# Chen-Suyi/PointRegGPT

Measured on AMD Instinct MI355X. Metric: generated point-cloud pairs/sec (node), 128x128 depth, 1000-step DDNM, higher is better.
Workload: dtype bf16; 1 GPU; configs[2]: full pipeline (SE(3) z-buffer reproject + MaskUnet + DDNM sampler + MaskUnet + f64 unproject); batch_per_gpu=64, image_size=128, transitions=1000, sampler=ancestral-ddnm, unet_dim=64, streams=2, parallelism=scene-sharded x1, no collectives, hipgraph=one captured transition (U-Net + update), replayed per step

## Files before the change

### include/prg.h

```cpp
#ifndef PRG_H
#define PRG_H

#include <stddef.h>
#include <stdint.h>

#ifdef __cplusplus
extern "C" {
#endif

#define PRG_ABI_VERSION 1

enum {
  PRG_OK = 0,
  PRG_E_INVALID = -1,
  PRG_E_HIP = -2,
  PRG_E_NOMEM = -3,
  PRG_E_STATE = -4
};

enum { PRG_F32 = 0, PRG_BF16 = 1, PRG_MXFP8 = 2, PRG_F16X3 = 3 };

int prg_abi_version(void);
const char* prg_last_error(void);
int prg_device_info(char* name, size_t name_len, int* compute_units);


int prg_depth2pc(const float* depth, const float* K, float* pc, uint8_t* valid, int B, int H, int W,
                 float clip_lo, float clip_hi, float invalid_value, void* stream);

int prg_pc2depth(const float* pc, const uint8_t* valid, const float* K, float* depth, uint8_t* mask,
                 int B, int N, int H, int W, void* stream);

int prg_project_points_zbuffer(const float* points, const int64_t* offsets, const float* pose, const float* K,
                               float* depth, uint8_t* mask, int B, int H, int W, float depth_scale,
                               void* stream);

int prg_reproject_zbuffer(const float* depth, const float* K, const float* pose, float* depth_out,
                          uint8_t* mask_out, int B, int H, int W, float depth_unit, float clip_lo,
                          float clip_hi, float out_scale, void* stream);

int prg_unproject_f64(const float* depth, const float* K, const float* pose, double* xyz, uint8_t* valid,
                      int B, int H, int W, float depth_unit, float clip_lo, float clip_hi, void* stream);

int prg_depth_augment(const float* depth, float* out, int B, int H, int W, void* stream);

int prg_apply_mask(const float* prob, const float* depth, const uint8_t* hit, float thr, float* depth_out,
                   uint8_t* hit_out, float* img_cond, int B, int H, int W, void* stream);

int prg_occlusion_filter(const float* depth, const uint8_t* mask, float* out, int B, int H, int W, float threshold,
                         void* stream);

int prg_overlap_counts(const double* pts, const int64_t* offsets, int n_pairs, int64_t max_cloud, double radius,
                       int32_t* counts, void* stream);

size_t prg_voxel_grid_workspace_bytes(int64_t total, int B);

int prg_voxel_grid_ragged(const double* pts, const uint8_t* valid, const int64_t* offsets, int B, int64_t total,
                          double voxel, double* out, int64_t* out_offsets, int32_t* status, void* workspace,
                          size_t workspace_bytes, void* stream);

int prg_merge_memory_f64(const float* memory, const int64_t* memory_offsets, int64_t memory_rows, const double* xyz,
                         const uint8_t* valid, int B, int HW, double* merged, uint8_t* merged_valid,
                         int64_t* merged_offsets, void* stream);


typedef struct prg_unet prg_unet;

typedef struct prg_unet_config {
  int32_t dim;
  int32_t n_levels;
  int32_t dim_mults[8];
  int32_t in_channels;
  int32_t conditional;
  int32_t param_cond_dim;
  int32_t groups;
  int32_t sigmoid_out;
} prg_unet_config;

int64_t prg_unet_param_count(const prg_unet_config* cfg);

int prg_unet_create(const prg_unet_config* cfg, const float* weights, int64_t n_floats, int dtype,
                    prg_unet** out);
int prg_unet_destroy(prg_unet* h);
int prg_unet_set_time_freqs(prg_unet* h, const float* freqs, int n);
int prg_unet_reserve(prg_unet* h, int B, int S);

int prg_unet_forward(prg_unet* h, const float* x, const int64_t* time, const float* param_cond, float* out,
                     int B, int S, void* stream);
int prg_maskunet_forward(prg_unet* h, const float* depth, float* prob, int B, int S, void* stream);

int prg_unet_set_taps(prg_unet* h, int enable);
int prg_unet_get_tap(prg_unet* h, const char* name, float* out, int64_t out_capacity_floats, int* C, int* H,
                     int* W, void* stream);

int prg_debug_conv3x3(const float* x, const float* w, const float* bias, float* out, int B, int Cin, int Cout, int H, int W,
                      int dtype, void* stream);
int prg_debug_block_pair(const float* x, const float* w1, const float* b1, const float* gamma, const float* beta, const float* w2,
                         const float* b2, float* out, int B, int Cin, int C, int H, int W, int groups, int h16, void* stream);
int prg_debug_upsample_conv3x3(const float* x, const float* w, const float* bias, float* out, int B, int Cin, int Cout, int H,
                               int W, void* stream);
int prg_debug_conv4x4s2(const float* x, const float* w, const float* bias, float* out, int B, int Cin, int Cout, int H, int W,
                        void* stream);
int prg_debug_conv(const float* x, const float* w, const float* bias, float* out, int B, int Cin, int Cout, int H, int W,
                   int dtype, int K, int stride, void* stream);
int prg_debug_upsample_conv(const float* x, const float* w, const float* bias, float* out, int B, int Cin, int Cout, int H, int W,
                            int dtype, void* stream);


typedef struct prg_sampler prg_sampler;

typedef struct prg_step {
  int32_t t;
  int32_t clip_pred;
  float c_x0, c_x, c_eps, sigma;
  float sqrt_recip, sqrt_recipm1;
} prg_step;

int prg_sampler_create(prg_unet* unet, const prg_step* steps, int n_steps, int B, int S, prg_sampler** out);
int prg_sampler_destroy(prg_sampler* h);
int prg_sampler_set_graph(prg_sampler* h, int enable);

int prg_sampler_run(prg_sampler* h, const float* param_cond, const float* img_cond, const float* noise,
                    int64_t noise_slabs, const uint64_t* seeds, float* out, void* stream);

int prg_debug_sampler_step(float* x, const float* u, const float* img_cond, const uint64_t* seeds, const prg_step* step, int B,
                           int HW, int reps, float* avg_us, void* stream);

int prg_sampler_set_profile(prg_sampler* h, int enable);
int prg_sampler_get_profile(prg_sampler* h, double* conv_ms, int64_t* conv_launches, double* conv_flops,
                            double* total_ms);
int prg_sampler_get_profile_bytes(prg_sampler* h, double* conv_bytes);
int prg_sampler_get_profile_executed(prg_sampler* h, double* conv_flops_executed);
typedef struct prg_profile_shape {
  int32_t cin, cout, k, stride, ups, hout, wout;
  int32_t two_source, prologue;
  int32_t mx;
  int64_t launches;
  double ms, flops, flops_executed;
} prg_profile_shape;
int prg_sampler_get_profile_shapes(prg_sampler* h, prg_profile_shape* rows, int32_t max_rows, int32_t* n_rows);
int prg_sampler_get_profile_step(prg_sampler* h, double* step_ms, int64_t* step_launches);


int prg_host_crop_aabb(const double* pts, int64_t n, const double* lo, const double* hi, double* out, int64_t* n_out);
int prg_host_voxel_down_sample(const double* pts, int64_t n, double voxel, double* out, int64_t* n_out);
int prg_host_write_ply(const char* path, const double* pts, int64_t n);

typedef struct prg_pool prg_pool;
int prg_pool_create(int n_threads, prg_pool** out);
int prg_pool_destroy(prg_pool* p);
int prg_pool_wait(prg_pool* p, int64_t* jobs_done);
int prg_pool_submit_cloud(prg_pool* p, const char* path, const double* xyz, int64_t n, const uint8_t* valid,
                          const double* T_pre, int crop, const double* lo, const double* hi, double voxel,
                          const double* T_post);
int prg_pool_submit_image(prg_pool* p, const char* path, const float* img, int H, int W, int kind);
int prg_pool_submit_text(prg_pool* p, const char* path, const double* values, int rows, int cols);

#ifdef __cplusplus
}
#endif
#endif
```

### pointreggpt_amd/_lib.py

```python
from __future__ import annotations

import ctypes as C
import os
from pathlib import Path

_HERE = Path(__file__).resolve().parent
LIB_PATH = Path(os.environ.get("PRG_HIP_LIB", _HERE / "libprg_hip.so"))

PRG_F32, PRG_BF16, PRG_MXFP8, PRG_F16X3 = 0, 1, 2, 3


class PrgError(RuntimeError):
    pass


class UnetConfigC(C.Structure):
    _fields_ = [("dim", C.c_int32), ("n_levels", C.c_int32), ("dim_mults", C.c_int32 * 8),
                ("in_channels", C.c_int32), ("conditional", C.c_int32), ("param_cond_dim", C.c_int32),
                ("groups", C.c_int32), ("sigmoid_out", C.c_int32)]


class StepC(C.Structure):
    _fields_ = [("t", C.c_int32), ("clip_pred", C.c_int32), ("c_x0", C.c_float), ("c_x", C.c_float),
                ("c_eps", C.c_float), ("sigma", C.c_float), ("sqrt_recip", C.c_float),
                ("sqrt_recipm1", C.c_float)]


_P, _I, _F, _L = C.c_void_p, C.c_int, C.c_float, C.c_int64

PROTOTYPES = {
    "prg_abi_version": (C.c_int, []),
    "prg_last_error": (C.c_char_p, []),
    "prg_device_info": (C.c_int, [C.c_char_p, C.c_size_t, C.POINTER(C.c_int)]),
    "prg_depth2pc": (C.c_int, [_P, _P, _P, _P, _I, _I, _I, _F, _F, _F, _P]),
    "prg_pc2depth": (C.c_int, [_P, _P, _P, _P, _P, _I, _I, _I, _I, _P]),
    "prg_project_points_zbuffer": (C.c_int, [_P, _P, _P, _P, _P, _P, _I, _I, _I, _F, _P]),
    "prg_reproject_zbuffer": (C.c_int, [_P, _P, _P, _P, _P, _I, _I, _I, _F, _F, _F, _F, _P]),
    "prg_unproject_f64": (C.c_int, [_P, _P, _P, _P, _P, _I, _I, _I, _F, _F, _F, _P]),
    "prg_depth_augment": (C.c_int, [_P, _P, _I, _I, _I, _P]),
    "prg_apply_mask": (C.c_int, [_P, _P, _P, _F, _P, _P, _P, _I, _I, _I, _P]),
    "prg_occlusion_filter": (C.c_int, [_P, _P, _P, _I, _I, _I, _F, _P]),
    "prg_overlap_counts": (C.c_int, [_P, _P, _I, _L, C.c_double, _P, _P]),
    "prg_voxel_grid_workspace_bytes": (C.c_size_t, [_L, _I]),
    "prg_voxel_grid_ragged": (C.c_int, [_P, _P, _P, _I, _L, C.c_double, _P, _P, _P, _P, C.c_size_t, _P]),
    "prg_merge_memory_f64": (C.c_int, [_P, _P, _L, _P, _P, _I, _I, _P, _P, _P, _P]),
    "prg_unet_param_count": (_L, [C.POINTER(UnetConfigC)]),
    "prg_unet_create": (C.c_int, [C.POINTER(UnetConfigC), _P, _L, _I, C.POINTER(_P)]),
    "prg_unet_destroy": (C.c_int, [_P]),
    "prg_unet_reserve": (C.c_int, [_P, _I, _I]),
    "prg_unet_set_time_freqs": (C.c_int, [_P, _P, _I]),
    "prg_unet_forward": (C.c_int, [_P, _P, _P, _P, _P, _I, _I, _P]),
    "prg_maskunet_forward": (C.c_int, [_P, _P, _P, _I, _I, _P]),
    "prg_debug_conv3x3": (C.c_int, [_P, _P, _P, _P, _I, _I, _I, _I, _I, _I, _P]),
    "prg_debug_block_pair": (C.c_int, [_P, _P, _P, _P, _P, _P, _P, _P, _I, _I, _I, _I, _I, _I, _I, _P]),
    "prg_debug_upsample_conv3x3": (C.c_int, [_P, _P, _P, _P, _I, _I, _I, _I, _I, _P]),
    "prg_debug_conv4x4s2": (C.c_int, [_P, _P, _P, _P, _I, _I, _I, _I, _I, _P]),
    "prg_debug_conv": (C.c_int, [_P, _P, _P, _P, _I, _I, _I, _I, _I, _I, _I, _I, _P]),
    "prg_debug_upsample_conv": (C.c_int, [_P, _P, _P, _P, _I, _I, _I, _I, _I, _I, _P]),
    "prg_unet_set_taps": (C.c_int, [_P, _I]),
    "prg_unet_get_tap": (C.c_int, [_P, C.c_char_p, _P, _L, C.POINTER(_I), C.POINTER(_I), C.POINTER(_I), _P]),
    "prg_sampler_create": (C.c_int, [_P, C.POINTER(StepC), _I, _I, _I, C.POINTER(_P)]),
    "prg_sampler_destroy": (C.c_int, [_P]),
    "prg_sampler_set_graph": (C.c_int, [_P, _I]),
    "prg_sampler_run": (C.c_int, [_P, _P, _P, _P, _L, _P, _P, _P]),
    "prg_sampler_set_profile": (C.c_int, [_P, _I]),
    "prg_sampler_get_profile": (C.c_int, [_P, C.POINTER(C.c_double), C.POINTER(_L), C.POINTER(C.c_double),
                                          C.POINTER(C.c_double)]),
    "prg_sampler_get_profile_bytes": (C.c_int, [_P, C.POINTER(C.c_double)]),
    "prg_sampler_get_profile_executed": (C.c_int, [_P, C.POINTER(C.c_double)]),
    "prg_sampler_get_profile_step": (C.c_int, [_P, C.POINTER(C.c_double), C.POINTER(_L)]),
    "prg_debug_sampler_step": (C.c_int, [_P, _P, _P, _P, _P, C.c_int, C.c_int, C.c_int, C.POINTER(C.c_float), _P]),
    "prg_sampler_get_profile_shapes": (C.c_int, [_P, _P, _I, C.POINTER(C.c_int32)]),
    "prg_host_crop_aabb": (C.c_int, [_P, _L, _P, _P, _P, C.POINTER(_L)]),
    "prg_host_voxel_down_sample": (C.c_int, [_P, _L, C.c_double, _P, C.POINTER(_L)]),
    "prg_host_write_ply": (C.c_int, [C.c_char_p, _P, _L]),
    "prg_pool_create": (C.c_int, [_I, C.POINTER(_P)]),
    "prg_pool_destroy": (C.c_int, [_P]),
    "prg_pool_wait": (C.c_int, [_P, C.POINTER(_L)]),
    "prg_pool_submit_cloud": (C.c_int, [_P, C.c_char_p, _P, _L, _P, _P, _I, _P, _P, C.c_double, _P]),
    "prg_pool_submit_image": (C.c_int, [_P, C.c_char_p, _P, _I, _I, _I]),
    "prg_pool_submit_text": (C.c_int, [_P, C.c_char_p, _P, _I, _I]),
}

_lib = None


def load():
    global _lib
    if _lib is not None:
        return _lib
    import torch
    if not LIB_PATH.exists():
        raise PrgError(f"{LIB_PATH} not found: build it with `python -c 'import __graft_entry__ as g; g.build()'` "
                       f"or `make -C pointreggpt_amd/csrc` (there is no CPU fallback)")
    try:
        lib = C.CDLL(str(LIB_PATH))
    except OSError as e:
        raise PrgError(f"cannot load {LIB_PATH}: {e}") from e
    lenient = os.environ.get("PRG_HIP_LIB_ALLOW_MISSING", "0") not in ("", "0") and bool(os.environ.get("PRG_HIP_LIB"))
    for name, (res, args) in PROTOTYPES.items():
        if lenient and not hasattr(lib, name):
            continue
        fn = getattr(lib, name)
        fn.restype = res
        fn.argtypes = args
    if lib.prg_abi_version() != 1:
        raise PrgError(f"ABI version mismatch: library {lib.prg_abi_version()}, binding 1")
    _lib = lib
    return lib


def check(rc: int, what: str = ""):
    if rc != 0:
        msg = load().prg_last_error()
        raise PrgError(f"{what or 'libprg_hip'} failed ({rc}): {msg.decode() if msg else ''}")


def ptr(t):
    if t is None:
        return None
    assert t.is_contiguous(), "tensor must be contiguous"
    return C.c_void_p(t.data_ptr())


def stream_ptr():
    import torch
    return C.c_void_p(torch.cuda.current_stream().cuda_stream)


def require_gpu():
    import torch
    if not torch.cuda.is_available():
        raise PrgError("no HIP device visible: pointreggpt_amd has no CPU path")
```

### pointreggpt_amd/csrc/attn_fused.hip

```cpp
#include <atomic>
#include <cstdlib>
#include <type_traits>

#include "blocks.h"

namespace prg {

typedef __attribute__((ext_vector_type(8))) __bf16 bf16x8;
typedef __attribute__((ext_vector_type(16))) float f32x16;
typedef __attribute__((ext_vector_type(2))) float f32x2;

namespace {

constexpr int kTP = 64;
constexpr int kHid = 128;
constexpr int kTilesPerBlock = 8;
constexpr int kLaCtxTpb = 8, kLaOutTpb = 8;
__host__ __device__ inline int la_tpb(int ntiles) {
  const int t = ntiles / 8;
  return t < 1 ? 1 : (t > kLaCtxTpb ? kLaCtxTpb : t);
}
__host__ __device__ inline int la_out_tpb(int ntiles) {
  const int t = ntiles / 8;
  return t < 1 ? 1 : (t > kLaOutTpb ? kLaOutTpb : t);
}
constexpr int kLdO = kHid + 8;
constexpr float kLnEps = 1e-5f;

__device__ inline uint32_t pack2(float a, float b) {
  typedef __attribute__((ext_vector_type(2))) __bf16 bf16x2;
  bf16x2 v = {(__bf16)a, (__bf16)b};
  return __builtin_bit_cast(uint32_t, v);
}
__device__ inline float bf_lo(uint32_t w) { return __uint_as_float(w << 16); }
__device__ inline float bf_hi(uint32_t w) { return __uint_as_float(w & 0xffff0000u); }
__device__ inline float fast_exp(float x) { return __builtin_amdgcn_exp2f(x * 1.4426950408889634f); }

template <int C>
struct Geo {
  static constexpr int LDW = C + 8;
  static constexpr int VPT = C / 32;
  static constexpr int KK = C / 16;
};

__device__ inline float quad_sum(float v) {
  v += __builtin_bit_cast(float, __builtin_amdgcn_mov_dpp(__builtin_bit_cast(int, v), 0xB1, 0xF, 0xF, true));
  v += __builtin_bit_cast(float, __builtin_amdgcn_mov_dpp(__builtin_bit_cast(int, v), 0x4E, 0xF, 0xF, true));
  return v;
}

template <int C>
struct XTile {
  uint4 v[Geo<C>::VPT];
  __device__ inline void load(const bf16_t* x, int64_t pix0, int valid) {
    const int row = threadIdx.x >> 2, part = threadIdx.x & 3;
#pragma unroll
    for (int i = 0; i < Geo<C>::VPT; ++i)
      v[i] = row < valid ? *reinterpret_cast<const uint4*>(x + (pix0 + row) * C + (part + 4 * i) * 8) : make_uint4(0, 0, 0, 0);
  }
  __device__ inline void normalize_to(__bf16* xn) const {
    const int row = threadIdx.x >> 2, part = threadIdx.x & 3;
    float f[Geo<C>::VPT][8];
    float s = 0.0f;
#pragma unroll
    for (int i = 0; i < Geo<C>::VPT; ++i) {
      const uint32_t w[4] = {v[i].x, v[i].y, v[i].z, v[i].w};
#pragma unroll
      for (int j = 0; j < 4; ++j) {
        f[i][2 * j] = bf_lo(w[j]);
        f[i][2 * j + 1] = bf_hi(w[j]);
        s += f[i][2 * j] + f[i][2 * j + 1];
      }
    }
    s = quad_sum(s);
    const float mean = s * (1.0f / C);
    float q = 0.0f;
#pragma unroll
    for (int i = 0; i < Geo<C>::VPT; ++i)
#pragma unroll
      for (int j = 0; j < 8; ++j) {
        f[i][j] -= mean;
        q = fmaf(f[i][j], f[i][j], q);
      }
    q = quad_sum(q);
    const float rstd = __builtin_amdgcn_rsqf(q * (1.0f / C) + kLnEps);
#pragma unroll
    for (int i = 0; i < Geo<C>::VPT; ++i) {
      uint4 o;
      o.x = pack2(f[i][0] * rstd, f[i][1] * rstd);
      o.y = pack2(f[i][2] * rstd, f[i][3] * rstd);
      o.z = pack2(f[i][4] * rstd, f[i][5] * rstd);
      o.w = pack2(f[i][6] * rstd, f[i][7] * rstd);
      *reinterpret_cast<uint4*>(xn + row * Geo<C>::LDW + (part + 4 * i) * 8) = o;
    }
  }
};

template <int COLS, int LD>
__device__ inline void stage_rows(__bf16* dst, const bf16_t* src, int nrows) {
  constexpr int VR = COLS / 8;
  for (int i = threadIdx.x; i < nrows * VR; i += 256) {
    const int r = i / VR, v = i - r * VR;
    *reinterpret_cast<uint4*>(dst + r * LD + v * 8) = *reinterpret_cast<const uint4*>(src + (size_t)r * COLS + v * 8);
  }
}

__device__ inline bf16x8 frag(const __bf16* rows, int ld, int l31, int hi, int kk) {
  return *reinterpret_cast<const bf16x8*>(rows + l31 * ld + kk * 16 + hi * 8);
}

template <int COLS>
__device__ inline void load_wfrags(bf16x8 (&w)[COLS / 16], const bf16_t* mat, int r0, int l31, int hi) {
#pragma unroll
  for (int kk = 0; kk < COLS / 16; ++kk)
    w[kk] = *reinterpret_cast<const bf16x8*>(mat + (size_t)(r0 + l31) * COLS + kk * 16 + hi * 8);
}

__device__ inline f32x16 zero16() {
  f32x16 z;
#pragma unroll
  for (int e = 0; e < 16; ++e) z[e] = 0.0f;
  return z;
}

template <int C>
__global__ __launch_bounds__(256) void la_kmax_fused_kernel(const bf16_t* __restrict__ x, const bf16_t* __restrict__ wqkv,
                                                            float* __restrict__ pmax, int N, int nslab) {
  using G = Geo<C>;
  extern __shared__ __attribute__((aligned(16))) char smem[];
  __bf16* xn = reinterpret_cast<__bf16*>(smem);
  const int b = blockIdx.y, slab = blockIdx.x;
  const int wave = threadIdx.x >> 6, lane = threadIdx.x & 63, l31 = lane & 31, hi = lane >> 5;
  const int ntiles = (N + kTP - 1) / kTP;
  const int tpb = la_tpb(ntiles), t0 = slab * tpb, t1 = min(t0 + tpb, ntiles);
  bf16x8 wk[G::KK];
  load_wfrags<C>(wk, wqkv, kHid + 32 * wave, l31, hi);
  float m = -INFINITY;
  XTile<C> xt;
  if (t0 < t1) xt.load(x, (int64_t)b * N + (int64_t)t0 * kTP, min(kTP, N - t0 * kTP));
  for (int t = t0; t < t1; ++t) {
    xt.normalize_to(xn);
    __syncthreads();
    if (t + 1 < t1) xt.load(x, (int64_t)b * N + (int64_t)(t + 1) * kTP, min(kTP, N - (t + 1) * kTP));
    f32x16 acc[2] = {zero16(), zero16()};
#pragma unroll
    for (int kk = 0; kk < G::KK; ++kk) {
#pragma unroll
      for (int pt = 0; pt < 2; ++pt)
        acc[pt] = __builtin_amdgcn_mfma_f32_32x32x16_bf16(frag(xn + pt * 32 * G::LDW, G::LDW, l31, hi, kk), wk[kk], acc[pt], 0, 0, 0);
    }
    const int valid = min(kTP, N - t * kTP);
#pragma unroll
    for (int pt = 0; pt < 2; ++pt)
#pragma unroll
      for (int r = 0; r < 16; ++r) {
        const int px = pt * 32 + (r & 3) + 8 * (r >> 2) + 4 * hi;
        if (px < valid) m = fmaxf(m, acc[pt][r]);
      }
    __syncthreads();
  }
  m = fmaxf(m, __shfl_xor(m, 32, 64));
  if (hi == 0) pmax[((size_t)b * nslab + slab) * kHid + 32 * wave + l31] = m;
}

template <int C, bool PSUM_MFMA, bool KSTAT>
__global__ __launch_bounds__(256, C == 64 ? 3 : (C == 128 ? 2 : 1)) void la_ctx_fused_kernel(const bf16_t* __restrict__ x, const bf16_t* __restrict__ wqkv,
                                                           const float* __restrict__ pmax, float* __restrict__ ctxp,
                                                           float* __restrict__ sump, int N, int nslab) {
  using G = Geo<C>;
  extern __shared__ __attribute__((aligned(16))) char smem[];
  __bf16* xn = reinterpret_cast<__bf16*>(smem);
  const int b = blockIdx.y, slab = blockIdx.x;
  const int wave = threadIdx.x >> 6, lane = threadIdx.x & 63, l31 = lane & 31, hi = lane >> 5;
  const int ntiles = (N + kTP - 1) / kTP;
  const int tpb = la_tpb(ntiles), t0 = slab * tpb, t1 = min(t0 + tpb, ntiles);
  bf16x8 wk[G::KK], wv[G::KK];
  load_wfrags<C>(wk, wqkv, kHid + 32 * wave, l31, hi);
  load_wfrags<C>(wv, wqkv, 2 * kHid + 32 * wave, l31, hi);
  f32x16 kinit0 = zero16();
  if constexpr (!KSTAT) {
    float m = -INFINITY;
    for (int s2 = 0; s2 < nslab; ++s2) m = fmaxf(m, pmax[((size_t)b * nslab + s2) * kHid + 32 * wave + l31]);
#pragma unroll
    for (int e = 0; e < 16; ++e) kinit0[e] = -m;
  }
  f32x16 ctx = zero16();
  f32x16 psum = zero16();
  float ssum = 0.0f;
  bf16x8 ones;
#pragma unroll
  for (int e = 0; e < 8; ++e) ones[e] = (__bf16)1.0f;
  XTile<C> xt;
  if (t0 < t1) xt.load(x, (int64_t)b * N + (int64_t)t0 * kTP, min(kTP, N - t0 * kTP));
  for (int t = t0; t < t1; ++t) {
    xt.normalize_to(xn);
    __syncthreads();
    if (t + 1 < t1) xt.load(x, (int64_t)b * N + (int64_t)(t + 1) * kTP, min(kTP, N - (t + 1) * kTP));
    const int valid = min(kTP, N - t * kTP);
    auto half = [&](const int pt, auto full_c) {
      constexpr bool FULL = decltype(full_c)::value;
      f32x16 k1, v1;
#pragma unroll
      for (int kk = 0; kk < G::KK; ++kk) {
        const bf16x8 xf = frag(xn + pt * 32 * G::LDW, G::LDW, l31, hi, kk);
        k1 = __builtin_amdgcn_mfma_f32_32x32x16_bf16(xf, wk[kk], kk == 0 ? (KSTAT ? zero16() : kinit0) : k1, 0, 0, 0);
        v1 = __builtin_amdgcn_mfma_f32_32x32x16_bf16(xf, wv[kk], kk == 0 ? zero16() : v1, 0, 0, 0);
      }
#pragma unroll
      for (int i = 0; i < 2; ++i) {
        bf16x8 pa, vb;
#pragma unroll
        for (int s2 = 0; s2 < 8; ++s2) {
          const int r = 8 * i + s2;
          float pe = __builtin_amdgcn_exp2f(k1[r]);
          if constexpr (!FULL) pe = (pt * 32 + (r & 3) + 8 * (r >> 2) + 4 * hi) < valid ? pe : 0.0f;
          if constexpr (!PSUM_MFMA) ssum += pe;
          pa[s2] = (__bf16)pe;
          vb[s2] = (__bf16)v1[r];
        }
        ctx = __builtin_amdgcn_mfma_f32_32x32x16_bf16(pa, vb, ctx, 0, 0, 0);
        if constexpr (PSUM_MFMA) psum = __builtin_amdgcn_mfma_f32_32x32x16_bf16(pa, ones, psum, 0, 0, 0);
      }
    };
    if (valid == kTP) {
      half(0, std::true_type{});
      half(1, std::true_type{});
    } else {
      half(0, std::false_type{});
      half(1, std::false_type{});
    }
    __syncthreads();
  }
  const size_t ph = ((size_t)b * 4 + wave) * nslab + slab;
  if constexpr (PSUM_MFMA) {
    if (l31 == 0) {
#pragma unroll
      for (int r = 0; r < 16; ++r) sump[ph * 32 + (r & 3) + 8 * (r >> 2) + 4 * hi] = psum[r];
    }
  } else {
    ssum += __shfl_xor(ssum, 32, 64);
    if (hi == 0) sump[ph * 32 + l31] = ssum;
  }
#pragma unroll
  for (int r = 0; r < 16; ++r) ctxp[ph * 1024 + ((r & 3) + 8 * (r >> 2) + 4 * hi) * 32 + l31] = ctx[r];
}

__global__ __launch_bounds__(256) void la_fin_fused_kernel(const float* __restrict__ ctxp, const float* __restrict__ sump,
                                                           bf16_t* __restrict__ ctxT, int N, int nslab) {
  const int h = blockIdx.x, b = blockIdx.y;
  const size_t ph = ((size_t)b * 4 + h) * nslab;
  const float scale = 0.17677669529663687f / (float)N;
  for (int idx = threadIdx.x; idx < 1024; idx += 256) {
    const int d = idx >> 5, e = idx & 31;
    float c = 0.0f, s = 0.0f;
    int s2 = 0;
    for (; s2 + 8 <= nslab; s2 += 8) {
      float cv[8], sv[8];
#pragma unroll
      for (int u = 0; u < 8; ++u) {
        cv[u] = ctxp[(ph + s2 + u) * 1024 + idx];
        sv[u] = sump[(ph + s2 + u) * 32 + d];
      }
#pragma unroll
      for (int u = 0; u < 8; ++u) {
        c += cv[u];
        s += sv[u];
      }
    }
    for (; s2 < nslab; ++s2) {
      c += ctxp[(ph + s2) * 1024 + idx];
      s += sump[(ph + s2) * 32 + d];
    }
    const int slot = (d >> 4) * 16 + ((d >> 2) & 1) * 8 + ((d >> 3) & 1) * 4 + (d & 3);
    ctxT[((size_t)b * 4 + h) * 1024 + e * 32 + slot] = f32_to_bf16(c / s * scale);
  }
}

template <int C, bool QSTAT>
__global__ __launch_bounds__(256, C == 64 ? 3 : (C == 128 ? 2 : 1)) void la_out_fused_kernel(const bf16_t* __restrict__ x, const bf16_t* __restrict__ wqkv,
                                                           const bf16_t* __restrict__ wout, const float* __restrict__ bias,
                                                           const float* __restrict__ out_g, const bf16_t* __restrict__ ctxT,
                                                           bf16_t* __restrict__ out, int N, const float* __restrict__ qshift) {
  using G = Geo<C>;
  constexpr int RT = C / 32;
  constexpr int NA = RT / 2;
  constexpr int NR = RT > 4 ? RT / 4 : 1;
  constexpr int RTL = RT > 4 ? RT : 4;
  extern __shared__ __attribute__((aligned(16))) char smem[];
  __bf16* xn = reinterpret_cast<__bf16*>(smem);
  __bf16* ot = xn + kTP * G::LDW;
  float* lnb = reinterpret_cast<float*>(ot + kTP * kLdO);
  __bf16* yt = reinterpret_cast<__bf16*>(lnb + kTP * RTL * 2);
  float* bias_l = reinterpret_cast<float*>(yt + kTP * G::LDW);
  float* outg_l = bias_l + C;
  if (threadIdx.x < C) {
    bias_l[threadIdx.x] = bias[threadIdx.x];
    outg_l[threadIdx.x] = out_g[threadIdx.x];
  }
  const int b = blockIdx.y, slab = blockIdx.x;
  const int wave = threadIdx.x >> 6, lane = threadIdx.x & 63, l31 = lane & 31, hi = lane >> 5;
  const int ntiles = (N + kTP - 1) / kTP;
  const int tpb = la_out_tpb(ntiles), t0 = slab * tpb, t1 = min(t0 + tpb, ntiles);
  bf16x8 wq[G::KK];
  load_wfrags<C>(wq, wqkv, 32 * wave, l31, hi);
  bf16x8 ca[2];
#pragma unroll
  for (int i = 0; i < 2; ++i)
    ca[i] = *reinterpret_cast<const bf16x8*>(ctxT + (((size_t)b * 4 + wave) * 32 + l31) * 32 + i * 16 + hi * 8);
  int yrt[NA], ypt[NA];
#pragma unroll
  for (int a = 0; a < NA; ++a) {
    if (RT == 2) { yrt[a] = wave & 1; ypt[a] = wave >> 1; }
    else if (RT <= 4) { yrt[a] = wave; ypt[a] = a; }
    else { yrt[a] = wave * NR + (a >> 1); ypt[a] = a & 1; }
  }
  bf16x8 wo[NR][kHid / 16];
#pragma unroll
  for (int r = 0; r < NR; ++r) load_wfrags<kHid>(wo[r], wout, yrt[RT > 4 ? 2 * r : 0] * 32, l31, hi);
  XTile<C> xt;
  if (t0 < t1) xt.load(x, (int64_t)b * N + (int64_t)t0 * kTP, min(kTP, N - t0 * kTP));
  for (int t = t0; t < t1; ++t) {
    asm volatile("" ::: "memory");
    const XTile<C> xraw = xt;
    const int valid = min(kTP, N - t * kTP);
    xt.normalize_to(xn);
    __syncthreads();
    if (t + 1 < t1) xt.load(x, (int64_t)b * N + (int64_t)(t + 1) * kTP, min(kTP, N - (t + 1) * kTP));
    constexpr bool qstat = QSTAT;
    f32x16 qa[2];
#pragma unroll
    for (int kk = 0; kk < G::KK; ++kk) {
#pragma unroll
      for (int pt = 0; pt < 2; ++pt)
        qa[pt] = __builtin_amdgcn_mfma_f32_32x32x16_bf16(wq[kk], frag(xn + pt * 32 * G::LDW, G::LDW, l31, hi, kk),
                                                         kk == 0 ? zero16() : qa[pt], 0, 0, 0);
    }
#pragma unroll
    for (int pt = 0; pt < 2; ++pt) {
      f32x16 oa = zero16();
      if constexpr (qstat) {
        f32x16 sa = zero16();
        bf16x8 ones;
#pragma unroll
        for (int e = 0; e < 8; ++e) ones[e] = (__bf16)1.0f;
#pragma unroll
        for (int i = 0; i < 2; ++i) {
          bf16x8 qb;
#pragma unroll
          for (int s2 = 0; s2 < 8; ++s2) qb[s2] = (__bf16)__builtin_amdgcn_exp2f(qa[pt][8 * i + s2]);
          oa = __builtin_amdgcn_mfma_f32_32x32x16_bf16(ca[i], qb, oa, 0, 0, 0);
          sa = __builtin_amdgcn_mfma_f32_32x32x16_bf16(ones, qb, sa, 0, 0, 0);
        }
        const float inv = __builtin_amdgcn_rcpf(sa[0]);
        const f32x2 inv2 = {inv, inv};
#pragma unroll
        for (int r = 0; r < 16; r += 2) {
          const f32x2 o2 = f32x2{oa[r], oa[r + 1]} * inv2;
          oa[r] = o2[0];
          oa[r + 1] = o2[1];
        }
      } else {
        float mx = qa[pt][0];
#pragma unroll
        for (int r = 1; r < 16; ++r) mx = fmaxf(mx, qa[pt][r]);
        mx = fmaxf(mx, __shfl_xor(mx, 32, 64));
        float sm = 0.0f;
#pragma unroll
        for (int r = 0; r < 16; ++r) {
          qa[pt][r] = __builtin_amdgcn_exp2f(qa[pt][r] - mx);
          sm += qa[pt][r];
        }
        sm += __shfl_xor(sm, 32, 64);
        const float inv = 1.0f / sm;
#pragma unroll
        for (int i = 0; i < 2; ++i) {
          bf16x8 qb;
#pragma unroll
          for (int s2 = 0; s2 < 8; ++s2) qb[s2] = (__bf16)(qa[pt][8 * i + s2] * inv);
          oa = __builtin_amdgcn_mfma_f32_32x32x16_bf16(ca[i], qb, oa, 0, 0, 0);
        }
      }
      const int px = pt * 32 + l31;
#pragma unroll
      for (int g4 = 0; g4 < 4; ++g4) {
        uint2 w;
        w.x = pack2(oa[4 * g4], oa[4 * g4 + 1]);
        w.y = pack2(oa[4 * g4 + 2], oa[4 * g4 + 3]);
        *reinterpret_cast<uint2*>(ot + px * kLdO + 32 * wave + 8 * g4 + 4 * hi) = w;
      }
    }
    __syncthreads();
    f32x16 ya[NA];
#pragma unroll
    for (int a = 0; a < NA; ++a) ya[a] = zero16();
#pragma unroll
    for (int kk = 0; kk < kHid / 16; ++kk) {
#pragma unroll
      for (int a = 0; a < NA; ++a)
        ya[a] = __builtin_amdgcn_mfma_f32_32x32x16_bf16(wo[RT > 4 ? (a >> 1) : 0][kk],
                                                        frag(ot + ypt[a] * 32 * kLdO, kLdO, l31, hi, kk), ya[a], 0, 0, 0);
    }
#pragma unroll
    for (int a = 0; a < NA; ++a) {
      float s1 = 0.0f, s2 = 0.0f;
#pragma unroll
      for (int r = 0; r < 16; ++r) {
        const int c = yrt[a] * 32 + (r & 3) + 8 * (r >> 2) + 4 * hi;
        ya[a][r] += bias_l[c];
        s1 += ya[a][r];
        s2 = fmaf(ya[a][r], ya[a][r], s2);
      }
      const auto sw = __builtin_amdgcn_permlane32_swap(__builtin_bit_cast(unsigned, s1), __builtin_bit_cast(unsigned, s2), false, false);
      const float tot = __builtin_bit_cast(float, (unsigned)sw[0]) + __builtin_bit_cast(float, (unsigned)sw[1]);
      lnb[((ypt[a] * 32 + l31) * RTL + yrt[a]) * 2 + hi] = tot;
    }
    __syncthreads();
#pragma unroll
    for (int a = 0; a < NA; ++a) {
      const int px = ypt[a] * 32 + l31;
      float s1 = 0.0f, s2 = 0.0f;
#pragma unroll
      for (int rt = 0; rt < RT; ++rt) {
        s1 += lnb[(px * RTL + rt) * 2];
        s2 += lnb[(px * RTL + rt) * 2 + 1];
      }
      const float mean = s1 * (1.0f / C);
      const float rstd = __builtin_amdgcn_rsqf(fmaxf(s2 * (1.0f / C) - mean * mean, 0.0f) + kLnEps);
#pragma unroll
      for (int g4 = 0; g4 < 4; ++g4) {
        const int c0 = yrt[a] * 32 + 8 * g4 + 4 * hi;
        const float4 gg = *reinterpret_cast<const float4*>(outg_l + c0);
        uint2 w;
        w.x = pack2((ya[a][4 * g4] - mean) * rstd * gg.x, (ya[a][4 * g4 + 1] - mean) * rstd * gg.y);
        w.y = pack2((ya[a][4 * g4 + 2] - mean) * rstd * gg.z, (ya[a][4 * g4 + 3] - mean) * rstd * gg.w);
        *reinterpret_cast<uint2*>(yt + px * G::LDW + c0) = w;
      }
    }
    __syncthreads();
    {
      const int row = threadIdx.x >> 2, part = threadIdx.x & 3;
      if (row < valid) {
#pragma unroll
        for (int i = 0; i < G::VPT; ++i) {
          const uint4 yv = *reinterpret_cast<const uint4*>(yt + row * G::LDW + (part + 4 * i) * 8);
          const uint4 xv = xraw.v[i];
          uint4 o;
          o.x = pack2(bf_lo(yv.x) + bf_lo(xv.x), bf_hi(yv.x) + bf_hi(xv.x));
          o.y = pack2(bf_lo(yv.y) + bf_lo(xv.y), bf_hi(yv.y) + bf_hi(xv.y));
          o.z = pack2(bf_lo(yv.z) + bf_lo(xv.z), bf_hi(yv.z) + bf_hi(xv.z));
          o.w = pack2(bf_lo(yv.w) + bf_lo(xv.w), bf_hi(yv.w) + bf_hi(xv.w));
          *reinterpret_cast<uint4*>(out + ((int64_t)b * N + (int64_t)t * kTP + row) * C + (part + 4 * i) * 8) = o;
        }
      }
    }
  }
}

template <int NT>
__global__ __launch_bounds__(256) void full_attn_mfma_kernel(const bf16_t* __restrict__ qkv, bf16_t* __restrict__ out) {
  constexpr int N = 32 * NT, LDK = 40, LDV = N + 8;
  __shared__ __attribute__((aligned(16))) __bf16 Ks[N * LDK];
  __shared__ __attribute__((aligned(16))) __bf16 Vt[32 * LDV];
  const int h = blockIdx.x, b = blockIdx.y, tid = threadIdx.x;
  const int wave = tid >> 6, lane = tid & 63, l31 = lane & 31, hi = lane >> 5;
  const bf16_t* base = qkv + (size_t)b * N * 384;
  for (int i = tid; i < N * 4; i += 256) {
    const int key = i >> 2, u = i & 3;
    *reinterpret_cast<uint4*>(Ks + key * LDK + u * 8) =
        *reinterpret_cast<const uint4*>(base + (size_t)key * 384 + 128 + h * 32 + u * 8);
    const uint4 vv = *reinterpret_cast<const uint4*>(base + (size_t)key * 384 + 256 + h * 32 + u * 8);
    const int d = key & 31;
    const int pos = (key & ~31) + (d >> 4) * 16 + ((d >> 2) & 1) * 8 + ((d >> 3) & 1) * 4 + (d & 3);
    const uint32_t w[4] = {vv.x, vv.y, vv.z, vv.w};
#pragma unroll
    for (int j = 0; j < 4; ++j) {
      reinterpret_cast<uint16_t*>(Vt)[(u * 8 + 2 * j) * LDV + pos] = (uint16_t)(w[j] & 0xffffu);
      reinterpret_cast<uint16_t*>(Vt)[(u * 8 + 2 * j + 1) * LDV + pos] = (uint16_t)(w[j] >> 16);
    }
  }
  __syncthreads();
  for (int qt = wave; qt < NT; qt += 4) {
    const bf16_t* qp = base + (size_t)(qt * 32 + l31) * 384 + h * 32 + hi * 8;
    const bf16x8 q0 = *reinterpret_cast<const bf16x8*>(qp), q1 = *reinterpret_cast<const bf16x8*>(qp + 16);
    f32x16 sacc[NT];
    float m = -INFINITY;
#pragma unroll
    for (int kt = 0; kt < NT; ++kt) {
      sacc[kt] = zero16();
      sacc[kt] = __builtin_amdgcn_mfma_f32_32x32x16_bf16(frag(Ks + kt * 32 * LDK, LDK, l31, hi, 0), q0, sacc[kt], 0, 0, 0);
      sacc[kt] = __builtin_amdgcn_mfma_f32_32x32x16_bf16(frag(Ks + kt * 32 * LDK, LDK, l31, hi, 1), q1, sacc[kt], 0, 0, 0);
#pragma unroll
      for (int r = 0; r < 16; ++r) {
        sacc[kt][r] *= 0.17677669529663687f;
        m = fmaxf(m, sacc[kt][r]);
      }
    }
    m = fmaxf(m, __shfl_xor(m, 32, 64));
    float l = 0.0f;
    f32x16 oacc = zero16();
#pragma unroll
    for (int kt = 0; kt < NT; ++kt) {
#pragma unroll
      for (int i = 0; i < 2; ++i) {
        bf16x8 pb;
#pragma unroll
        for (int s2 = 0; s2 < 8; ++s2) {
          const float pv = fast_exp(sacc[kt][8 * i + s2] - m);
          l += pv;
          pb[s2] = (__bf16)pv;
        }
        oacc = __builtin_amdgcn_mfma_f32_32x32x16_bf16(
            *reinterpret_cast<const bf16x8*>(Vt + l31 * LDV + kt * 32 + i * 16 + hi * 8), pb, oacc, 0, 0, 0);
      }
    }
    l += __shfl_xor(l, 32, 64);
    const float inv = 1.0f / l;
    bf16_t* op = out + ((size_t)b * N + qt * 32 + l31) * 128 + h * 32 + 4 * hi;
#pragma unroll
    for (int g4 = 0; g4 < 4; ++g4) {
      uint2 w;
      w.x = pack2(oacc[4 * g4] * inv, oacc[4 * g4 + 1] * inv);
      w.y = pack2(oacc[4 * g4 + 2] * inv, oacc[4 * g4 + 3] * inv);
      *reinterpret_cast<uint2*>(op + 8 * g4) = w;
    }
  }
}


template <int NT, int QS>
__global__ __launch_bounds__(256) void full_attn_mfma_big_kernel(const bf16_t* __restrict__ qkv, bf16_t* __restrict__ out) {
  constexpr int N = 32 * NT, LDK = 40, LDV = N + 8;
  extern __shared__ __attribute__((aligned(16))) char smem_attn[];
  __bf16* Ks = reinterpret_cast<__bf16*>(smem_attn);
  __bf16* Vt = Ks + N * LDK;
  const int h = blockIdx.x, b = blockIdx.y, qs = blockIdx.z, tid = threadIdx.x;
  const int wave = tid >> 6, lane = tid & 63, l31 = lane & 31, hi = lane >> 5;
  const bf16_t* base = qkv + (size_t)b * N * 384;
  for (int i = tid; i < N * 4; i += 256) {
    const int key = i >> 2, u = i & 3;
    *reinterpret_cast<uint4*>(Ks + key * LDK + u * 8) =
        *reinterpret_cast<const uint4*>(base + (size_t)key * 384 + 128 + h * 32 + u * 8);
    const uint4 vv = *reinterpret_cast<const uint4*>(base + (size_t)key * 384 + 256 + h * 32 + u * 8);
    const int d = key & 31;
    const int pos = (key & ~31) + (d >> 4) * 16 + ((d >> 2) & 1) * 8 + ((d >> 3) & 1) * 4 + (d & 3);
    const uint32_t w[4] = {vv.x, vv.y, vv.z, vv.w};
#pragma unroll
    for (int j = 0; j < 4; ++j) {
      reinterpret_cast<uint16_t*>(Vt)[(u * 8 + 2 * j) * LDV + pos] = (uint16_t)(w[j] & 0xffffu);
      reinterpret_cast<uint16_t*>(Vt)[(u * 8 + 2 * j + 1) * LDV + pos] = (uint16_t)(w[j] >> 16);
    }
  }
  __syncthreads();
  for (int qt = qs * 4 + wave; qt < NT; qt += 4 * QS) {
    const bf16_t* qp = base + (size_t)(qt * 32 + l31) * 384 + h * 32 + hi * 8;
    const bf16x8 q0 = *reinterpret_cast<const bf16x8*>(qp), q1 = *reinterpret_cast<const bf16x8*>(qp + 16);
    float m = -INFINITY;
#pragma unroll 2
    for (int kt = 0; kt < NT; ++kt) {
      f32x16 sa = zero16();
      sa = __builtin_amdgcn_mfma_f32_32x32x16_bf16(frag(Ks + kt * 32 * LDK, LDK, l31, hi, 0), q0, sa, 0, 0, 0);
      sa = __builtin_amdgcn_mfma_f32_32x32x16_bf16(frag(Ks + kt * 32 * LDK, LDK, l31, hi, 1), q1, sa, 0, 0, 0);
#pragma unroll
      for (int r = 0; r < 16; ++r) m = fmaxf(m, sa[r] * 0.17677669529663687f);
    }
    m = fmaxf(m, __shfl_xor(m, 32, 64));
    float l = 0.0f;
    f32x16 oacc = zero16();
#pragma unroll 2
    for (int kt = 0; kt < NT; ++kt) {
      f32x16 sa = zero16();
      sa = __builtin_amdgcn_mfma_f32_32x32x16_bf16(frag(Ks + kt * 32 * LDK, LDK, l31, hi, 0), q0, sa, 0, 0, 0);
      sa = __builtin_amdgcn_mfma_f32_32x32x16_bf16(frag(Ks + kt * 32 * LDK, LDK, l31, hi, 1), q1, sa, 0, 0, 0);
#pragma unroll
      for (int i = 0; i < 2; ++i) {
        bf16x8 pb;
#pragma unroll
        for (int s2 = 0; s2 < 8; ++s2) {
          const float pv = fast_exp(sa[8 * i + s2] * 0.17677669529663687f - m);
          l += pv;
          pb[s2] = (__bf16)pv;
        }
        oacc = __builtin_amdgcn_mfma_f32_32x32x16_bf16(
            *reinterpret_cast<const bf16x8*>(Vt + l31 * LDV + kt * 32 + i * 16 + hi * 8), pb, oacc, 0, 0, 0);
      }
    }
    l += __shfl_xor(l, 32, 64);
    const float inv = 1.0f / l;
    bf16_t* op = out + ((size_t)b * N + qt * 32 + l31) * 128 + h * 32 + 4 * hi;
#pragma unroll
    for (int g4 = 0; g4 < 4; ++g4) {
      uint2 w;
      w.x = pack2(oacc[4 * g4] * inv, oacc[4 * g4 + 1] * inv);
      w.y = pack2(oacc[4 * g4 + 2] * inv, oacc[4 * g4 + 3] * inv);
      *reinterpret_cast<uint2*>(op + 8 * g4) = w;
    }
  }
}

template <int C>
size_t lds_kmax() { return (size_t)kTP * Geo<C>::LDW * 2; }
template <int C>
size_t lds_out() { return (size_t)2 * kTP * Geo<C>::LDW * 2 + (size_t)kTP * kLdO * 2 + (size_t)kTP * (C / 32 > 4 ? C / 32 : 4) * 2 * 4 + (size_t)2 * C * 4; }

template <typename K>
int set_lds(K kernel, size_t bytes) {
  hipError_t e = hipFuncSetAttribute(reinterpret_cast<const void*>(kernel), hipFuncAttributeMaxDynamicSharedMemorySize, (int)bytes);
  if (e != hipSuccess) return fail(PRG_E_HIP, std::string("hipFuncSetAttribute(fused attention): ") + hipGetErrorString(e));
  return PRG_OK;
}

int la_slabs(int N) { const int nt = ceil_div(N, kTP); return ceil_div(nt, la_tpb(nt)); }
int tail_slabs(int N) { return ceil_div(ceil_div(N, kTP), kTilesPerBlock); }

template <int CIN, int COUT>
__global__ __launch_bounds__(256) void resblock_tail_fused_kernel(const bf16_t* __restrict__ h, const float* __restrict__ A,
                                                                  const float* __restrict__ Bc, const bf16_t* __restrict__ s0,
                                                                  int C0, const bf16_t* __restrict__ s1, int C1,
                                                                  const bf16_t* __restrict__ wres, const float* __restrict__ bres,
                                                                  bf16_t* __restrict__ out, int N, const float* __restrict__ head_w,
                                                                  const float* __restrict__ head_b, float* __restrict__ head_out,
                                                                  int head_sigmoid, const GnFold fold) {
  constexpr int LDX = CIN + 8, LDH = COUT + 8;
  constexpr int RT = COUT / 32, NA = RT / 2;
  constexpr int XV = CIN / 32, HV = COUT / 32;
  extern __shared__ __attribute__((aligned(16))) char smem[];
  __bf16* xs = reinterpret_cast<__bf16*>(smem);
  __bf16* hs = xs + kTP * LDX;
  const int b = blockIdx.y, slab = blockIdx.x;
  const int wave = threadIdx.x >> 6, lane = threadIdx.x & 63, l31 = lane & 31, hi = lane >> 5;
  const int row = threadIdx.x >> 2, part = threadIdx.x & 3;
  const int ntiles = (N + kTP - 1) / kTP;
  const int t0 = slab * kTilesPerBlock, t1 = min(t0 + kTilesPerBlock, ntiles);
  const int yrt = RT == 2 ? (wave & 1) : wave;
  int ypt[NA];
#pragma unroll
  for (int a = 0; a < NA; ++a) ypt[a] = RT == 2 ? (wave >> 1) : a;
  bf16x8 wr[CIN / 16];
  load_wfrags<CIN>(wr, wres, yrt * 32, l31, hi);
  float4 ca[4], cb[4], cr[4];
#pragma unroll
  for (int g4 = 0; g4 < 4; ++g4) {
    const int c0 = yrt * 32 + 8 * g4 + 4 * hi;
    if (fold.acc) {
      float mean, rstd;
      gn_fold_stats(fold, b, c0 / fold.cpg, mean, rstd);
      const float4 p4 = *reinterpret_cast<const float4*>(fold.P + (size_t)b * fold.pq_stride + c0);
      const float4 q4 = *reinterpret_cast<const float4*>(fold.Q + (size_t)b * fold.pq_stride + c0);
      ca[g4] = make_float4(rstd * p4.x, rstd * p4.y, rstd * p4.z, rstd * p4.w);
      cb[g4] = make_float4(fmaf(-mean, ca[g4].x, q4.x), fmaf(-mean, ca[g4].y, q4.y), fmaf(-mean, ca[g4].z, q4.z),
                           fmaf(-mean, ca[g4].w, q4.w));
    } else {
      ca[g4] = *reinterpret_cast<const float4*>(A + (size_t)b * COUT + c0);
      cb[g4] = *reinterpret_cast<const float4*>(Bc + (size_t)b * COUT + c0);
    }
    cr[g4] = *reinterpret_cast<const float4*>(bres + c0);
  }
  uint4 xv[XV], hv[HV];
  auto load_tile = [&](int t) {
    const int valid = min(kTP, N - t * kTP);
    const int64_t pix = (int64_t)b * N + (int64_t)t * kTP + row;
#pragma unroll
    for (int i = 0; i < XV; ++i) {
      const int c = (part + 4 * i) * 8;
      xv[i] = row < valid ? (c < C0 ? *reinterpret_cast<const uint4*>(s0 + pix * C0 + c)
                                    : *reinterpret_cast<const uint4*>(s1 + pix * C1 + (c - C0)))
                          : make_uint4(0, 0, 0, 0);
    }
#pragma unroll
    for (int i = 0; i < HV; ++i)
      hv[i] = row < valid ? *reinterpret_cast<const uint4*>(h + pix * COUT + (part + 4 * i) * 8) : make_uint4(0, 0, 0, 0);
  };
  if (t0 < t1) load_tile(t0);
  for (int t = t0; t < t1; ++t) {
    const int valid = min(kTP, N - t * kTP);
#pragma unroll
    for (int i = 0; i < XV; ++i) *reinterpret_cast<uint4*>(xs + row * LDX + (part + 4 * i) * 8) = xv[i];
#pragma unroll
    for (int i = 0; i < HV; ++i) *reinterpret_cast<uint4*>(hs + row * LDH + (part + 4 * i) * 8) = hv[i];
    __syncthreads();
    if (t + 1 < t1) load_tile(t + 1);
    f32x16 ya[NA];
#pragma unroll
    for (int a = 0; a < NA; ++a) ya[a] = zero16();
#pragma unroll
    for (int kk = 0; kk < CIN / 16; ++kk)
#pragma unroll
      for (int a = 0; a < NA; ++a)
        ya[a] = __builtin_amdgcn_mfma_f32_32x32x16_bf16(wr[kk], frag(xs + ypt[a] * 32 * LDX, LDX, l31, hi, kk), ya[a], 0, 0, 0);
#pragma unroll
    for (int a = 0; a < NA; ++a) {
      const int px = ypt[a] * 32 + l31;
#pragma unroll
      for (int g4 = 0; g4 < 4; ++g4) {
        __bf16* hp = hs + px * LDH + yrt * 32 + 8 * g4 + 4 * hi;
        const uint2 hw = *reinterpret_cast<const uint2*>(hp);
        const float a4[4] = {ca[g4].x, ca[g4].y, ca[g4].z, ca[g4].w};
        const float b4[4] = {cb[g4].x, cb[g4].y, cb[g4].z, cb[g4].w};
        const float r4[4] = {cr[g4].x, cr[g4].y, cr[g4].z, cr[g4].w};
        const float hx[4] = {bf_lo(hw.x), bf_hi(hw.x), bf_lo(hw.y), bf_hi(hw.y)};
        float y[4];
#pragma unroll
        for (int j = 0; j < 4; ++j) y[j] = Elem<bf16_t>::silu(fmaf(hx[j], a4[j], b4[j])) + (ya[a][4 * g4 + j] + r4[j]);
        uint2 w;
        w.x = pack2(y[0], y[1]);
        w.y = pack2(y[2], y[3]);
        *reinterpret_cast<uint2*>(hp) = w;
      }
    }
    __syncthreads();
    if (head_out) {
      float acc = 0.0f;
#pragma unroll
      for (int i = 0; i < HV; ++i) {
        const uint4 v = *reinterpret_cast<const uint4*>(hs + row * LDH + (part + 4 * i) * 8);
        const float* w = head_w + (part + 4 * i) * 8;
        const uint32_t q[4] = {v.x, v.y, v.z, v.w};
#pragma unroll
        for (int j = 0; j < 4; ++j) {
          acc = fmaf(bf_lo(q[j]), w[2 * j], acc);
          acc = fmaf(bf_hi(q[j]), w[2 * j + 1], acc);
        }
      }
      acc += __shfl_xor(acc, 1, 64);
      acc += __shfl_xor(acc, 2, 64);
      if (part == 0 && row < valid) {
        const float y = acc + head_b[0];
        head_out[(int64_t)b * N + (int64_t)t * kTP + row] = head_sigmoid ? 1.0f / (1.0f + expf(-y)) : y;
      }
    } else if (row < valid) {
#pragma unroll
      for (int i = 0; i < HV; ++i)
        *reinterpret_cast<uint4*>(out + ((int64_t)b * N + (int64_t)t * kTP + row) * COUT + (part + 4 * i) * 8) =
            *reinterpret_cast<const uint4*>(hs + row * LDH + (part + 4 * i) * 8);
    }
    __syncthreads();
  }
}

template <int CIN, int COUT>
int launch_tail(const bf16_t* h, const float* A, const float* Bc, const bf16_t* s0, int C0, const bf16_t* s1, int C1,
                const bf16_t* wres, const float* bres, bf16_t* out, int B, int N, hipStream_t s, const GnFold& fold,
                const float* head_w = nullptr, const float* head_b = nullptr, float* head_out = nullptr, int head_sigmoid = 0) {
  const size_t lds = (size_t)kTP * (CIN + 8 + COUT + 8) * 2;
  static DeviceOnce attr;
  if (!attr.done()) {
    int rc = set_lds(&resblock_tail_fused_kernel<CIN, COUT>, lds);
    if (rc) return rc;
    attr.mark();
  }
  resblock_tail_fused_kernel<CIN, COUT><<<dim3(tail_slabs(N), B), 256, lds, s>>>(h, A, Bc, s0, C0, s1, C1, wres, bres, out, N, head_w, head_b,
                                                                                 head_out, head_sigmoid, fold);
  PRG_LAUNCH_CHECK();
  return PRG_OK;
}


template <int C>
constexpr bool kPsumDefault = C >= 128;

template <int C>
int launch_c(const bf16_t* x, const bf16_t* wqkv, const bf16_t* wout, const float* bias, const float* out_g, bf16_t* out,
             float* ws, int B, int N, const float* kshift, hipStream_t s) {
  static DeviceOnce attr;
  if (!attr.done()) {
    int rc;
    if ((rc = set_lds(&la_kmax_fused_kernel<C>, lds_kmax<C>()))) return rc;
    if ((rc = set_lds(&la_ctx_fused_kernel<C, false, false>, lds_kmax<C>()))) return rc;
    if ((rc = set_lds(&la_ctx_fused_kernel<C, false, true>, lds_kmax<C>()))) return rc;
    if ((rc = set_lds(&la_ctx_fused_kernel<C, true, false>, lds_kmax<C>()))) return rc;
    if ((rc = set_lds(&la_ctx_fused_kernel<C, true, true>, lds_kmax<C>()))) return rc;
    if ((rc = set_lds(&la_out_fused_kernel<C, false>, lds_out<C>()))) return rc;
    if ((rc = set_lds(&la_out_fused_kernel<C, true>, lds_out<C>()))) return rc;
    attr.mark();
  }
  const int nslab = la_slabs(N);
  float* pmax = ws;
  float* ctxp = pmax + (size_t)B * nslab * kHid;
  float* sump = ctxp + (size_t)B * 4 * nslab * 1024;
  bf16_t* ctxT = reinterpret_cast<bf16_t*>(sump + (size_t)B * 4 * nslab * 32);
  const dim3 grid(nslab, B);
  if (!kshift) {
    la_kmax_fused_kernel<C><<<grid, 256, lds_kmax<C>(), s>>>(x, wqkv, pmax, N, nslab);
    PRG_LAUNCH_CHECK();
  }
  static const int psum_env = env_int("PRG_LA_PSUM", -1);
  const bool psum = psum_env > 0 || (psum_env < 0 && kPsumDefault<C>);
#define PRG_LA_CTX_GO(PS, KS) la_ctx_fused_kernel<C, PS, KS><<<grid, 256, lds_kmax<C>(), s>>>(x, wqkv, pmax, ctxp, sump, N, nslab)
  if (kshift) { if (psum) PRG_LA_CTX_GO(true, true); else PRG_LA_CTX_GO(false, true); }
  else { if (psum) PRG_LA_CTX_GO(true, false); else PRG_LA_CTX_GO(false, false); }
#undef PRG_LA_CTX_GO
  PRG_LAUNCH_CHECK();
  la_fin_fused_kernel<<<dim3(4, B), 256, 0, s>>>(ctxp, sump, ctxT, N, nslab);
  PRG_LAUNCH_CHECK();
  const int nt = ceil_div(N, kTP);
  const dim3 ogrid(ceil_div(nt, la_out_tpb(nt)), B);
  if (kshift) la_out_fused_kernel<C, true><<<ogrid, 256, lds_out<C>(), s>>>(x, wqkv, wout, bias, out_g, ctxT, out, N, kshift + kHid);
  else la_out_fused_kernel<C, false><<<ogrid, 256, lds_out<C>(), s>>>(x, wqkv, wout, bias, out_g, ctxT, out, N, nullptr);
  PRG_LAUNCH_CHECK();
  return PRG_OK;
}

}

bool full_attention_mfma_supported(int N) { return N == 64 || N == 128 || N == 256 || N == 512 || N == 1024; }

template <int NT, int QS>
static int launch_attn_big(const bf16_t* qkv, bf16_t* out, int B, hipStream_t s) {
  constexpr int N = 32 * NT;
  constexpr size_t lds = ((size_t)N * 40 + (size_t)32 * (N + 8)) * 2;
  static DeviceOnce attr;
  if (!attr.done()) {
    int rc = set_lds(&full_attn_mfma_big_kernel<NT, QS>, lds);
    if (rc) return rc;
    attr.mark();
  }
  full_attn_mfma_big_kernel<NT, QS><<<dim3(4, B, QS), 256, lds, s>>>(qkv, out);
  PRG_LAUNCH_CHECK();
  return PRG_OK;
}

int launch_full_attention_mfma(const bf16_t* qkv, bf16_t* out, int B, int N, hipStream_t s) {
  PRG_CHECK(full_attention_mfma_supported(N) && qkv && out, "full attention (MFMA): unsupported token count");
  const dim3 grid(4, B);
  if (N == 1024) return B >= 32 ? launch_attn_big<32, 2>(qkv, out, B, s) : launch_attn_big<32, 4>(qkv, out, B, s);
  if (N == 512) return launch_attn_big<16, 2>(qkv, out, B, s);
  if (N == 64) full_attn_mfma_kernel<2><<<grid, 256, 0, s>>>(qkv, out);
  else if (N == 128) full_attn_mfma_kernel<4><<<grid, 256, 0, s>>>(qkv, out);
  else full_attn_mfma_kernel<8><<<grid, 256, 0, s>>>(qkv, out);
  PRG_LAUNCH_CHECK();
  return PRG_OK;
}

bool resblock_tail_fused_supported(int C0, int C1, int Cout) {
  const int cin = C0 + C1;
  return C0 % 8 == 0 && C1 % 8 == 0 && ((cin == 128 && Cout == 64) || (cin == 192 && Cout == 128) || (cin == 256 && Cout == 128));
}

int launch_resblock_tail_fused(const bf16_t* h, const float* A, const float* Bc, const bf16_t* s0, int C0, const bf16_t* s1,
                               int C1, const bf16_t* wres, const float* bres, bf16_t* out, int B, int N, int Cout,
                               hipStream_t s,
                               const float* head_w, const float* head_b, float* head_out, int head_sigmoid, const GnFold* fold) {
  PRG_CHECK(resblock_tail_fused_supported(C0, C1, Cout) && bres, "fused resblock tail: unsupported shape");
  PRG_CHECK(!head_out || (Cout == 64 && head_w && head_b), "fused resblock tail: the head needs Cout = 64");
  GnFold f{};
  if (fold && fold->acc) {
    f = *fold;
    PRG_CHECK(f.cpg % 4 == 0 && f.G * f.cpg == Cout && f.P && f.Q, "fused resblock tail: bad GroupNorm fold");
  } else {
    PRG_CHECK(A && Bc, "fused resblock tail: no coefficients");
  }
  if (Cout == 64) return launch_tail<128, 64>(h, A, Bc, s0, C0, s1, C1, wres, bres, out, B, N, s, f, head_w, head_b, head_out, head_sigmoid);
  if (C0 + C1 == 192) return launch_tail<192, 128>(h, A, Bc, s0, C0, s1, C1, wres, bres, out, B, N, s, f);
  return launch_tail<256, 128>(h, A, Bc, s0, C0, s1, C1, wres, bres, out, B, N, s, f);
}

bool linattn_fused_supported(int C) { return C == 64 || C == 128 || C == 256; }

size_t linattn_fused_ws_floats(int B, int N) {
  const size_t ns = la_slabs(N);
  return (size_t)B * ns * kHid + (size_t)B * 4 * ns * 1024 + (size_t)B * 4 * ns * 32 + (size_t)B * 4 * 1024 / 2 + 64;
}

int launch_linear_attention_fused(const bf16_t* x, const bf16_t* wqkv, const bf16_t* wout, const float* bias,
                                  const float* out_g, bf16_t* out, float* ws, int B, int N, int C, const float* kshift,
                                  hipStream_t s) {
  PRG_CHECK(linattn_fused_supported(C), "fused linear attention: unsupported width");
  PRG_CHECK(la_slabs(N) <= 4096, "fused linear attention: too many slabs");
  if (C == 64) return launch_c<64>(x, wqkv, wout, bias, out_g, out, ws, B, N, kshift, s);
  if (C == 256) return launch_c<256>(x, wqkv, wout, bias, out_g, out, ws, B, N, kshift, s);
  return launch_c<128>(x, wqkv, wout, bias, out_g, out, ws, B, N, kshift, s);
}

}
```

### pointreggpt_amd/csrc/conv.h

```cpp
#pragma once
#include <vector>

#include "common.h"

namespace prg {

template <typename T>
struct ConvTile {
  static constexpr int BK = 64 / (int)sizeof(T);
};

struct ConvDesc {
  int B, Hin, Win;
  int C0, C1;
  int ups;
  int KH, KW, stride, pad;
  int Hout, Wout;
  int Cout, CoutPad;
  int kchunks;
};

template <typename T>
void pack_conv_weight(const float* w_oihw, int Cout, int Cin, int KH, int KW, std::vector<T>& out, int* CoutPad,
                      int* kchunks);

template <typename T>
struct ConvLaunch {
  ConvDesc d;
  const T* src0;
  const T* src1;
  const T* w;
  const float* bias;
  const T* residual;
  const float* res_a;
  const float* res_b;
  T* out;
  float* gn_partials;
  int gn_groups;
  const float* pro_a;
  const float* pro_b;
  GnApply gn{};
  float* gn_coef_a = nullptr;
  float* gn_coef_b = nullptr;
  int* gn_tickets = nullptr;
  long long* gn_acc;
  GnFold pro_fold;
  GnFold res_fold;
  const uint8_t* w_mx;
  const uint8_t* w_mx_scale;
  int mx_pure;
  const T* w_s2d;
  int s2d_kchunks;
  const T* w_up = nullptr;
  const uint16_t* w_split;
  int split_kchunks;
  const uint16_t* w_up_split = nullptr;
  const float* split_scale = nullptr;
  const float* split_scale_up = nullptr;
  int out_f16 = 0, in_f16 = 0, probe = 0;
  const uint16_t* w_f16 = nullptr;
};

#if defined(__HIPCC__)
typedef __attribute__((ext_vector_type(2))) _Float16 h16x2;
__device__ inline uint32_t h16_pack(float a, float b) {
  typedef __attribute__((ext_vector_type(2))) float f32x2;
  const f32x2 p = {a, b};
  return __builtin_bit_cast(uint32_t, __builtin_convertvector(p, h16x2));
}
typedef __attribute__((ext_vector_type(4))) unsigned int h16_u32x4;
#define PRG_H16_TRANS4(OP)                                                                                             \
  asm(OP "_e32 %0, %4\n\t" OP "_e32 %1, %5\n\t" OP "_e32 %2, %6\n\t" OP "_e32 %3, %7\n\t"                            \
      OP "_sdwa %0, %4 dst_sel:WORD_1 dst_unused:UNUSED_PRESERVE src0_sel:WORD_1\n\t"                                  \
      OP "_sdwa %1, %5 dst_sel:WORD_1 dst_unused:UNUSED_PRESERVE src0_sel:WORD_1\n\t"                                  \
      OP "_sdwa %2, %6 dst_sel:WORD_1 dst_unused:UNUSED_PRESERVE src0_sel:WORD_1\n\t"                                  \
      OP "_sdwa %3, %7 dst_sel:WORD_1 dst_unused:UNUSED_PRESERVE src0_sel:WORD_1\n\ts_nop 0"                           \
      : "=&v"(o0), "=&v"(o1), "=&v"(o2), "=&v"(o3)                                                                      \
      : "v"(i0), "v"(i1), "v"(i2), "v"(i3))
__device__ inline h16_u32x4 h16_silu8(h16_u32x4 x, const h16x2 (&a)[4], const h16x2 (&b)[4]) {
  const h16x2 nl2e = {(_Float16)-1.4426950408889634f, (_Float16)-1.4426950408889634f}, one = {(_Float16)1.0f, (_Float16)1.0f};
  h16x2 y[4];
  uint32_t i0, i1, i2, i3, o0, o1, o2, o3;
#pragma unroll
  for (int j = 0; j < 4; ++j) {
    const uint32_t w = x[j];
    y[j] = __builtin_elementwise_fma(__builtin_bit_cast(h16x2, w), a[j], b[j]);
  }
  i0 = __builtin_bit_cast(uint32_t, y[0] * nl2e); i1 = __builtin_bit_cast(uint32_t, y[1] * nl2e);
  i2 = __builtin_bit_cast(uint32_t, y[2] * nl2e); i3 = __builtin_bit_cast(uint32_t, y[3] * nl2e);
  PRG_H16_TRANS4("v_exp_f16");
  i0 = __builtin_bit_cast(uint32_t, __builtin_bit_cast(h16x2, o0) + one); i1 = __builtin_bit_cast(uint32_t, __builtin_bit_cast(h16x2, o1) + one);
  i2 = __builtin_bit_cast(uint32_t, __builtin_bit_cast(h16x2, o2) + one); i3 = __builtin_bit_cast(uint32_t, __builtin_bit_cast(h16x2, o3) + one);
  PRG_H16_TRANS4("v_rcp_f16");
  h16_u32x4 r;
  r[0] = __builtin_bit_cast(uint32_t, y[0] * __builtin_bit_cast(h16x2, o0));
  r[1] = __builtin_bit_cast(uint32_t, y[1] * __builtin_bit_cast(h16x2, o1));
  r[2] = __builtin_bit_cast(uint32_t, y[2] * __builtin_bit_cast(h16x2, o2));
  r[3] = __builtin_bit_cast(uint32_t, y[3] * __builtin_bit_cast(h16x2, o3));
  return r;
}
#undef PRG_H16_TRANS4
#endif

void pack_conv_weight_f16(const float* w_oihw, int Cout, int Cin, int KH, int KW, std::vector<uint16_t>& out);
bool conv_h16_pair_ok(const ConvLaunch<bf16_t>& L1, const ConvLaunch<bf16_t>& L2);

void pack_conv_weight_split(const float* w_oihw, int Cout, int Cin, int KH, int KW, std::vector<uint16_t>& out, int* CoutPad,
                            int* kchunks32, std::vector<float>* oscale = nullptr);
int try_launch_conv_split(const ConvLaunch<float>& L, hipStream_t s, int* gn_nsplit_out);

void s2d_equivalent_weights(const float* w_oihw, int Cout, int Cin, std::vector<float>& out);
void up_equivalent_weights(const float* w_oihw, int Cout, int Cin, std::vector<float>& out);

void pack_conv_weight_mxfp8(const float* w_oihw, int Cout, int Cin, int KH, int KW, std::vector<uint8_t>& data,
                            std::vector<uint8_t>& scales, int* CoutPad, int* chunks64);
uint8_t f32_to_e4m3(float v);
float e4m3_to_f32(uint8_t b);

template <typename T>
int launch_conv(const ConvLaunch<T>& L, hipStream_t s, int* gn_nsplit_out, int* acc_done = nullptr);

template <typename T>
bool conv_supports_prologue(const ConvDesc& d);

double conv_last_exec_scale();
int conv_last_was_mx();

inline double conv_flops(const ConvDesc& d) {
  return 2.0 * (double)d.B * d.Hout * d.Wout * d.Cout * (double)(d.C0 + d.C1) * d.KH * d.KW;
}

bool stem_conv_mfma_supported(int Cin, int Cout, int H, int W);
int launch_stem_conv_mfma(const float* x, const bf16_t* wf, const float* bias, bf16_t* out, int B, int Cin, int H, int W, hipStream_t s);
void pack_stem_mfma_weights(const float* w, int Cin, std::vector<bf16_t>& out);
int launch_stem_conv_mfma_split(const float* x, const uint16_t* wf, const float* bias, const float* wscale, float* out, int B, int Cin,
                                int H, int W, hipStream_t s);
void pack_stem_mfma_weights_split(const float* w, int Cin, std::vector<uint16_t>& out, std::vector<float>& scale);
template <typename T>
int launch_stem_conv(const float* x, const float* wk, const float* bias, T* out, int B, int Cin, int H, int W,
                     int Cout, hipStream_t s);

template <typename T>
int launch_head_conv(const T* x, const float* w, const float* bias, float* out, int64_t M, int C, int sigmoid,
                     hipStream_t s);

}
```

### pointreggpt_amd/csrc/conv.hip

```cpp
#include <cmath>
#include <cstdio>
#include <cstring>
#include <type_traits>

#include "blocks.h"
#include "conv.h"
#include "conv_epi.h"

namespace prg {

template <typename T>
struct Mma;

template <>
struct Mma<bf16_t> {
  static constexpr int UNITS_PER_CALL = 2;
  using Frag = bf16x8;
  __device__ static inline int unit_of(int call, int hi) { return call * 2 + hi; }
  __device__ static inline Frag load(const void* p) { return *reinterpret_cast<const Frag*>(p); }
  __device__ static inline void mma(const Frag& a, const Frag& b, f32x16& c, int ) {
    c = __builtin_amdgcn_mfma_f32_32x32x16_bf16(a, b, c, 0, 0, 0);
  }
};

template <>
struct Mma<float> {
  static constexpr int UNITS_PER_CALL = 1;
  struct Frag {
    float4 v;
  };
  __device__ static inline int unit_of(int call, int ) { return call; }
  __device__ static inline Frag load(const void* p) {
    Frag f;
    f.v = *reinterpret_cast<const float4*>(p);
    return f;
  }
  __device__ static inline void mma(const Frag& a, const Frag& b, f32x16& c, int hi) {
    c = __builtin_amdgcn_mfma_f32_32x32x2f32(hi ? a.v.y : a.v.x, hi ? b.v.y : b.v.x, c, 0, 0, 0);
    c = __builtin_amdgcn_mfma_f32_32x32x2f32(hi ? a.v.w : a.v.z, hi ? b.v.w : b.v.z, c, 0, 0, 0);
  }
};


template <int TM>
__device__ inline void clear_acc(f32x16 (&acc)[TM][2]) {
#pragma unroll
  for (int i = 0; i < TM; ++i)
#pragma unroll
    for (int j = 0; j < 2; ++j)
#pragma unroll
      for (int e = 0; e < 16; ++e) acc[i][j][e] = 0.0f;
}
template <typename T, int TM = 1>
struct Wide {
  static constexpr bool on = false;
  __device__ inline void add(const f32x16 (&)[TM][2]) {}
  __device__ inline void finish(f32x16 (&)[TM][2]) {}
};
template <int TM>
struct Wide<float, TM> {
  static constexpr bool on = true;
  double tot[TM][2][16];
  __device__ inline Wide() {
#pragma unroll
    for (int i = 0; i < TM; ++i)
#pragma unroll
      for (int j = 0; j < 2; ++j)
#pragma unroll
        for (int e = 0; e < 16; ++e) tot[i][j][e] = 0.0;
  }
  __device__ inline void add(const f32x16 (&acc)[TM][2]) {
#pragma unroll
    for (int i = 0; i < TM; ++i)
#pragma unroll
      for (int j = 0; j < 2; ++j)
#pragma unroll
        for (int e = 0; e < 16; ++e) tot[i][j][e] += (double)acc[i][j][e];
  }
  __device__ inline void finish(f32x16 (&acc)[TM][2]) {
#pragma unroll
    for (int i = 0; i < TM; ++i)
#pragma unroll
      for (int j = 0; j < 2; ++j)
#pragma unroll
        for (int e = 0; e < 16; ++e) acc[i][j][e] = (float)tot[i][j][e];
  }
};

template <typename T, int TH, int TW, int BN>
__global__ __launch_bounds__(256, sizeof(T) == 4 ? 1 : 2) void conv3x3_halo_kernel(const ConvLaunch<T> L, const int tiles_x,
                                                           const int tiles_y, const int tiles_n, const int fuse_stats) {
  constexpr int VEC = Elem<T>::kVec;
  constexpr int CH = 8 * VEC;
  constexpr int BKG = ConvTile<T>::BK;
  constexpr int BM = TH * TW;
  constexpr int HP = TW + 2, HALO = (TH + 2) * HP;
  constexpr int NH = (HALO * 8 + 255) / 256;
  constexpr int NB = BN * 8 / 256;
  constexpr int WAVES_N = BN / 64, WAVES_M = 4 / WAVES_N;
  constexpr int WM = BM / WAVES_M, TM = WM / 32;
  constexpr int CALLS = 8 / Mma<T>::UNITS_PER_CALL;
  static_assert(WM % 32 == 0 && TM >= 1, "wave tile");

  extern __shared__ __attribute__((aligned(16))) char smem[];
  uint4* Ah = reinterpret_cast<uint4*>(smem);
  uint4* Bs = Ah + HALO * 8;
  float* stage = reinterpret_cast<float*>(smem);

  const ConvDesc& d = L.d;
  const int nblk = tiles_x * tiles_y * tiles_n * d.B;
  int lin = xcd_remap(blockIdx.x, nblk);
  const int tn = lin % tiles_n; lin /= tiles_n;
  const int tx = lin % tiles_x; lin /= tiles_x;
  const int ty = lin % tiles_y;
  const int b = lin / tiles_y;
  const int y0 = ty * TH, x0 = tx * TW;

  const int tid = threadIdx.x, wave = tid >> 6, lane = tid & 63;
  const int wm = wave / WAVES_N, wn = wave % WAVES_N;
  const int l31 = lane & 31, hi = lane >> 5;
  const int Cin = d.C0 + d.C1;
  const int nchunks = Cin / CH;
  const int Hl = d.Hout, Wl = d.Wout;
  const int slot = tid & 7;

  int64_t hsrc[NH];
#pragma unroll
  for (int k = 0; k < NH; ++k) {
    const int hp = (tid >> 3) + k * 32;
    hsrc[k] = -1;
    if (hp < HALO) {
      const int hy = hp / HP, hx = hp - hy * HP;
      int y = y0 - 1 + hy, x = x0 - 1 + hx;
      if ((unsigned)y < (unsigned)Hl && (unsigned)x < (unsigned)Wl) {
        if (d.ups) { y >>= 1; x >>= 1; }
        hsrc[k] = ((int64_t)b * d.Hin + y) * d.Win + x;
      }
    }
  }
  int ahp[TM];
#pragma unroll
  for (int i = 0; i < TM; ++i) {
    const int p = wm * WM + i * 32 + l31;
    ahp[i] = (p / TW) * HP + (p % TW);
  }

  Vec16<T> hreg[NH], breg[NB];
  auto gload_halo = [&](int chunk) {
    const int c = chunk * CH + slot * VEC;
    const bool first = c < d.C0;
    const T* base = first ? L.src0 : L.src1;
    const int Cs = first ? d.C0 : d.C1, cc = first ? c : c - d.C0;
#pragma unroll
    for (int k = 0; k < NH; ++k) hreg[k] = hsrc[k] >= 0 ? vec_load(base + hsrc[k] * Cs + cc) : vec_zero<T>();
  };
  auto gload_b = [&](int chunk, int tap) {
#pragma unroll
    for (int j = 0; j < NB; ++j) {
      const int n = (tid >> 3) + j * 32;
      const T* p = L.w + ((size_t)(tap * d.kchunks + 2 * chunk + (slot >> 2)) * d.CoutPad + tn * BN + n) * BKG +
                   (slot & 3) * VEC;
      breg[j] = vec_load(p);
    }
  };

  f32x16 acc[TM][2];
#pragma unroll
  for (int i = 0; i < TM; ++i)
#pragma unroll
    for (int j = 0; j < 2; ++j)
#pragma unroll
      for (int e = 0; e < 16; ++e) acc[i][j][e] = 0.0f;

  Wide<T, TM> wacc;
  const int niter = nchunks * 9;
  gload_halo(0);
  gload_b(0, 0);
  int tap = 0, chunk = 0;
  for (int it = 0; it < niter; ++it) {
    if (tap == 0) {
      if (it > 0) __syncthreads();
      float pa[VEC], pb[VEC];
      if (L.pro_a) {
#pragma unroll
        for (int u = 0; u < VEC; ++u) {
          pa[u] = L.pro_a[(size_t)b * d.C0 + chunk * CH + slot * VEC + u];
          pb[u] = L.pro_b[(size_t)b * d.C0 + chunk * CH + slot * VEC + u];
        }
      }
#pragma unroll
      for (int k = 0; k < NH; ++k) {
        const int hp = (tid >> 3) + k * 32;
        if (hp < HALO) {
          Vec16<T> v = hreg[k];
          if (L.pro_a && hsrc[k] >= 0) {
#pragma unroll
            for (int u = 0; u < VEC; ++u) v.e[u] = Elem<T>::store(Elem<T>::silu(fmaf(Elem<T>::load(v.e[u]), pa[u], pb[u])));
          }
          Ah[hp * 8 + (slot ^ ((hp >> 1) & 7))] = *reinterpret_cast<const uint4*>(&v);
        }
      }
    }
    uint4* Bb = Bs + (it & 1) * BN * 8;
#pragma unroll
    for (int j = 0; j < NB; ++j) {
      const int n = (tid >> 3) + j * 32;
      Bb[n * 8 + (slot ^ ((n >> 1) & 7))] = *reinterpret_cast<const uint4*>(&breg[j]);
    }
    __syncthreads();
    const int ntap = tap == 8 ? 0 : tap + 1, nchunk = tap == 8 ? chunk + 1 : chunk;
    if (it + 1 < niter) gload_b(nchunk, ntap);
    if (tap == 0 && chunk + 1 < nchunks) gload_halo(chunk + 1);

    const int kh = tap / 3, kw = tap - kh * 3;
    const int toff = kh * HP + kw;
    if constexpr (Wide<T>::on) clear_acc<TM>(acc);
#pragma unroll
    for (int call = 0; call < CALLS; ++call) {
      const int unit = Mma<T>::unit_of(call, hi);
      typename Mma<T>::Frag fa[TM], fb[2];
#pragma unroll
      for (int i = 0; i < TM; ++i) {
        const int hp = ahp[i] + toff;
        fa[i] = Mma<T>::load(Ah + hp * 8 + (unit ^ ((hp >> 1) & 7)));
      }
#pragma unroll
      for (int j = 0; j < 2; ++j) {
        const int n = wn * 64 + j * 32 + l31;
        fb[j] = Mma<T>::load(Bb + n * 8 + (unit ^ ((n >> 1) & 7)));
      }
#pragma unroll
      for (int i = 0; i < TM; ++i)
#pragma unroll
        for (int j = 0; j < 2; ++j) Mma<T>::mma(fa[i], fb[j], acc[i][j], hi);
    }
    wacc.add(acc);
    tap = ntap;
    chunk = nchunk;
  }
  wacc.finish(acc);

  StatAcc<T> gs, gq;
  auto row_to_m = [&](int r) -> int64_t {
    const int p = wm * WM + r;
    return ((int64_t)b * d.Hout + y0 + p / TW) * d.Wout + x0 + p % TW;
  };
  epilogue_store<T, TM>(L, acc, stage + wave * 32 * 68, lane, tn * BN + wn * 64, row_to_m, gs, gq);
  if (fuse_stats) {
    const int nsplit = tiles_x * tiles_y;
    float* dst = L.gn_partials + ((size_t)b * nsplit + ty * tiles_x + tx) * L.gn_groups * 2;
    epilogue_stats<WAVES_M, WAVES_N>(reinterpret_cast<StatAcc<T>*>(stage + 4 * 32 * 68), gs, gq, wave, lane, tn * BN, d.Cout,
                                     L.gn_groups, dst);
  }
}

typedef __attribute__((ext_vector_type(8))) int mx_i32x8;

__device__ inline uint32_t mx_cvt4(float a, float b, float c, float d) {
  int w = 0;
  w = __builtin_amdgcn_cvt_pk_fp8_f32(a, b, w, false);
  w = __builtin_amdgcn_cvt_pk_fp8_f32(c, d, w, true);
  return (uint32_t)w;
}

template <int TH, int TW, int BN>
__global__ __launch_bounds__(256, 2) void conv3x3_mx_kernel(const ConvLaunch<bf16_t> L, const int tiles_x, const int tiles_y,
                                                            const int tiles_n, const int fuse_stats) {
  using T = bf16_t;
  constexpr int CH = 64;
  constexpr int ROWB = 80;
  constexpr int BM = TH * TW;
  constexpr int HP = TW + 2, HALO = (TH + 2) * HP;
  constexpr int NH = (HALO * 8 + 255) / 256;
  constexpr int NB = BN * 4 / 256;
  constexpr int WAVES_N = BN / 64, WAVES_M = 4 / WAVES_N;
  constexpr int WM = BM / WAVES_M, TM = WM / 32;
  static_assert(WM % 32 == 0 && TM >= 1 && NB >= 1, "wave tile");

  extern __shared__ __attribute__((aligned(16))) char smem[];
  char* Ah = smem;
  char* Bw = Ah + HALO * ROWB;
  unsigned char* As = reinterpret_cast<unsigned char*>(Bw + 2 * BN * ROWB);
  unsigned char* Bsc = As + ((HALO * 2 + 15) & ~15);
  float* stage = reinterpret_cast<float*>(smem);

  const ConvDesc& d = L.d;
  const int nblk = tiles_x * tiles_y * tiles_n * d.B;
  int lin = xcd_remap(blockIdx.x, nblk);
  const int tn = lin % tiles_n; lin /= tiles_n;
  const int tx = lin % tiles_x; lin /= tiles_x;
  const int ty = lin % tiles_y;
  const int b = lin / tiles_y;
  const int y0 = ty * TH, x0 = tx * TW;
  const int tid = threadIdx.x, wave = tid >> 6, lane = tid & 63;
  const int wm = wave / WAVES_N, wn = wave % WAVES_N;
  const int l31 = lane & 31, hi = lane >> 5;
  const int nchunks = (d.C0 + d.C1) / CH;
  const int Hl = d.Hout, Wl = d.Wout;
  const int slot = tid & 7;

  int64_t hsrc[NH];
#pragma unroll
  for (int k = 0; k < NH; ++k) {
    const int hp = (tid >> 3) + k * 32;
    hsrc[k] = -1;
    if (hp < HALO) {
      const int hy = hp / HP, hx = hp - hy * HP;
      int y = y0 - 1 + hy, x = x0 - 1 + hx;
      if ((unsigned)y < (unsigned)Hl && (unsigned)x < (unsigned)Wl) {
        if (d.ups) { y >>= 1; x >>= 1; }
        hsrc[k] = ((int64_t)b * d.Hin + y) * d.Win + x;
      }
    }
  }
  int ahp[TM];
#pragma unroll
  for (int i = 0; i < TM; ++i) {
    const int p = wm * WM + i * 32 + l31;
    ahp[i] = (p / TW) * HP + (p % TW);
  }

  Vec16<T> hreg[NH];
  uint4 breg[NB];
  uint16_t bsreg = 0;
  auto gload_halo = [&](int chunk) {
    const int c = chunk * CH + slot * 8;
    const bool first = c < d.C0;
    const T* base = first ? L.src0 : L.src1;
    const int Cs = first ? d.C0 : d.C1, cc = first ? c : c - d.C0;
#pragma unroll
    for (int k = 0; k < NH; ++k) hreg[k] = hsrc[k] >= 0 ? vec_load(base + hsrc[k] * Cs + cc) : vec_zero<T>();
  };
  auto gload_b = [&](int chunk, int tap) {
    const size_t tile = (size_t)(tap * nchunks + chunk) * d.CoutPad + (size_t)tn * BN;
#pragma unroll
    for (int j = 0; j < NB; ++j) {
      const int u = tid + j * 256;
      breg[j] = *reinterpret_cast<const uint4*>(L.w_mx + (tile + (u >> 2)) * 64 + (u & 3) * 16);
    }
    if (tid < BN) bsreg = *reinterpret_cast<const uint16_t*>(L.w_mx_scale + (tile + tid) * 2);
  };

  f32x16 acc[TM][2];
#pragma unroll
  for (int i = 0; i < TM; ++i)
#pragma unroll
    for (int j = 0; j < 2; ++j)
#pragma unroll
      for (int e = 0; e < 16; ++e) acc[i][j][e] = 0.0f;

  const int niter = nchunks * 9;
  gload_halo(0);
  gload_b(0, 0);
  int tap = 0, chunk = 0;
  for (int it = 0; it < niter; ++it) {
    if (tap == 0) {
      if (it > 0) __syncthreads();
      float pa[8], pb[8];
      if (L.pro_a) {
#pragma unroll
        for (int u = 0; u < 8; ++u) {
          pa[u] = L.pro_a[(size_t)b * d.C0 + chunk * CH + slot * 8 + u];
          pb[u] = L.pro_b[(size_t)b * d.C0 + chunk * CH + slot * 8 + u];
        }
      }
#pragma unroll
      for (int k = 0; k < NH; ++k) {
        const int hp = (tid >> 3) + k * 32;
        if (hp < HALO) {
          float f[8];
#pragma unroll
          for (int u = 0; u < 8; ++u) f[u] = Elem<T>::load(hreg[k].e[u]);
          if (L.pro_a && hsrc[k] >= 0) {
#pragma unroll
            for (int u = 0; u < 8; ++u) f[u] = Elem<T>::load(Elem<T>::store(Elem<T>::silu(fmaf(f[u], pa[u], pb[u]))));
          }
          float am = 0.0f;
#pragma unroll
          for (int u = 0; u < 8; ++u) am = fmaxf(am, fabsf(f[u]));
          am = fmaxf(am, __shfl_xor(am, 1, 64));
          am = fmaxf(am, __shfl_xor(am, 2, 64));
          const int E = (int)((__float_as_uint(am) >> 23) & 0xffu);
          const int S = E > 8 ? E - 8 : 0;
          const float mult = __uint_as_float((uint32_t)(254 - S) << 23);
          float g[8];
#pragma unroll
          for (int u = 0; u < 8; ++u) g[u] = fminf(fmaxf(f[u] * mult, -448.0f), 448.0f);
          uint2 w;
          w.x = mx_cvt4(g[0], g[1], g[2], g[3]);
          w.y = mx_cvt4(g[4], g[5], g[6], g[7]);
          *reinterpret_cast<uint2*>(Ah + hp * ROWB + slot * 8) = w;
          if ((slot & 3) == 0) As[hp * 2 + (slot >> 2)] = (unsigned char)S;
        }
      }
    }
    char* Bb = Bw + (it & 1) * BN * ROWB;
    unsigned char* Sb = Bsc + (it & 1) * BN * 2;
#pragma unroll
    for (int j = 0; j < NB; ++j) {
      const int u = tid + j * 256;
      *reinterpret_cast<uint4*>(Bb + (u >> 2) * ROWB + (u & 3) * 16) = breg[j];
    }
    if (tid < BN) *reinterpret_cast<uint16_t*>(Sb + tid * 2) = bsreg;
    __syncthreads();
    const int ntap = tap == 8 ? 0 : tap + 1, nchunk = tap == 8 ? chunk + 1 : chunk;
    if (it + 1 < niter) gload_b(nchunk, ntap);
    if (tap == 0 && chunk + 1 < nchunks) gload_halo(chunk + 1);

    const int kh = tap / 3, kw = tap - kh * 3;
    const int toff = kh * HP + kw;
    mx_i32x8 fa[TM], fb[2];
    int sa[TM], sb[2];
#pragma unroll
    for (int i = 0; i < TM; ++i) {
      const int hp = ahp[i] + toff;
      const uint4 lo = *reinterpret_cast<const uint4*>(Ah + hp * ROWB + hi * 16);
      const uint4 up = *reinterpret_cast<const uint4*>(Ah + hp * ROWB + 32 + hi * 16);
      fa[i] = mx_i32x8{(int)lo.x, (int)lo.y, (int)lo.z, (int)lo.w, (int)up.x, (int)up.y, (int)up.z, (int)up.w};
      sa[i] = As[hp * 2 + hi];
    }
#pragma unroll
    for (int j = 0; j < 2; ++j) {
      const int n = wn * 64 + j * 32 + l31;
      const uint4 lo = *reinterpret_cast<const uint4*>(Bb + n * ROWB + hi * 16);
      const uint4 up = *reinterpret_cast<const uint4*>(Bb + n * ROWB + 32 + hi * 16);
      fb[j] = mx_i32x8{(int)lo.x, (int)lo.y, (int)lo.z, (int)lo.w, (int)up.x, (int)up.y, (int)up.z, (int)up.w};
      sb[j] = Sb[n * 2 + hi];
    }
#pragma unroll
    for (int i = 0; i < TM; ++i)
#pragma unroll
      for (int j = 0; j < 2; ++j)
        acc[i][j] = __builtin_amdgcn_mfma_scale_f32_32x32x64_f8f6f4(fa[i], fb[j], acc[i][j], 0, 0, 0, sa[i], 0, sb[j]);
    tap = ntap;
    chunk = nchunk;
  }

  StatAcc<T> gs, gq;
  auto row_to_m = [&](int r) -> int64_t {
    const int p = wm * WM + r;
    return ((int64_t)b * d.Hout + y0 + p / TW) * d.Wout + x0 + p % TW;
  };
  epilogue_store<T, TM>(L, acc, stage + wave * 32 * 68, lane, tn * BN + wn * 64, row_to_m, gs, gq);
  if (fuse_stats) {
    const int nsplit = tiles_x * tiles_y;
    float* dst = L.gn_partials + ((size_t)b * nsplit + ty * tiles_x + tx) * L.gn_groups * 2;
    epilogue_stats<WAVES_M, WAVES_N>(reinterpret_cast<StatAcc<T>*>(stage + 4 * 32 * 68), gs, gq, wave, lane, tn * BN, d.Cout,
                                     L.gn_groups, dst);
  }
}

template <typename T, int BM, int BN, bool ONE>
__global__ __launch_bounds__(256, sizeof(T) == 4 ? 1 : 2) void conv_igemm_kernel(const ConvLaunch<T> L, const int M, const int tiles_m,
                                                         const int tiles_n, const int fuse_stats, const int wide) {
  constexpr int BK = ConvTile<T>::BK;
  constexpr int VEC = Elem<T>::kVec;
  constexpr int UPR = BK / VEC;
  constexpr int RPP = 256 / UPR;
  constexpr int AP = BM / RPP, BP = BN / RPP;
  constexpr int WAVES_N = BN / 64, WAVES_M = 4 / WAVES_N;
  constexpr int WM = BM / WAVES_M, TM = WM / 32;
  constexpr int CALLS = UPR / Mma<T>::UNITS_PER_CALL;
  static_assert(TM >= 1, "wave tile");

  extern __shared__ __attribute__((aligned(16))) char smem[];
  uint4* As = reinterpret_cast<uint4*>(smem);
  uint4* Bs = As + 2 * BM * UPR;
  float* stage = reinterpret_cast<float*>(smem);
  constexpr int PITCH = UPR;
  static_assert(UPR == 4, "swizzle assumes 64-byte tile rows");

  const ConvDesc& d = L.d;
  const int lin = xcd_remap(blockIdx.x, tiles_m * tiles_n);
  const int tn = lin % tiles_n, tm = lin / tiles_n;

  const int tid = threadIdx.x;
  const int lrow = tid / UPR, ku = tid % UPR;
  const int Cin = d.C0 + d.C1;
  const int Hl = d.ups ? 2 * d.Hin : d.Hin, Wl = d.ups ? 2 * d.Win : d.Win;
  const int HWo = d.Hout * d.Wout;

  int a_iy0[AP], a_ix0[AP];
  int64_t a_base[AP];
  bool a_ok[AP];
  const T* a_p0[AP];
  const T* a_p1[AP];
#pragma unroll
  for (int i = 0; i < AP; ++i) {
    const int m = tm * BM + lrow + i * RPP;
    a_ok[i] = m < M;
    const int mm = a_ok[i] ? m : 0;
    if constexpr (ONE) {
      a_p0[i] = L.src0 + (int64_t)mm * d.C0 + ku * VEC;
      a_p1[i] = d.C1 ? L.src1 + (int64_t)mm * d.C1 + ku * VEC - d.C0 : a_p0[i];
    } else {
      const int bb = mm / HWo, rem = mm - bb * HWo;
      const int oy = rem / d.Wout, ox = rem - oy * d.Wout;
      a_iy0[i] = oy * d.stride - d.pad;
      a_ix0[i] = ox * d.stride - d.pad;
      a_base[i] = (int64_t)bb * d.Hin * d.Win;
    }
  }

  typedef __attribute__((ext_vector_type(4))) unsigned int stg_t;
  auto ldg = [](const T* p) { return *reinterpret_cast<const stg_t*>(p); };
  stg_t ra0[AP], rb0[BP], ra1[AP], rb1[BP];
  unsigned ok0 = 0, ok1 = 0;
  const int niter = d.KH * d.KW * d.kchunks;
  auto gload = [&](stg_t(&ra)[AP], stg_t(&rb)[BP], unsigned& okm, int tap, int kc) {
    okm = 0;
    const int kh = tap / d.KW, kw = tap - kh * d.KW;
    const int c = kc * BK + ku * VEC;
    if constexpr (ONE) {
#pragma unroll
      for (int i = 0; i < AP; ++i) {
        const bool ok = a_ok[i] && c < Cin;
        const T* p = (c < d.C0 ? a_p0[i] : a_p1[i]) + kc * BK;
        ra[i] = ldg(ok ? p : L.src0);
        okm |= (ok ? 1u : 0u) << i;
      }
    } else
#pragma unroll
    for (int i = 0; i < AP; ++i) {
      int iy = a_iy0[i] + kh, ix = a_ix0[i] + kw;
      const bool ok = a_ok[i] && (unsigned)iy < (unsigned)Hl && (unsigned)ix < (unsigned)Wl && c < Cin;
      if (d.ups) { iy >>= 1; ix >>= 1; }
      const int64_t pix = ok ? a_base[i] + (int64_t)iy * d.Win + ix : 0;
      const T* p = (c < d.C0) ? L.src0 + pix * d.C0 + c : L.src1 + pix * d.C1 + (c - d.C0);
      ra[i] = ldg(ok ? p : L.src0);
      okm |= (ok ? 1u : 0u) << i;
    }
    const T* wt = L.w + ((size_t)(tap * d.kchunks + kc) * d.CoutPad + (size_t)tn * BN) * BK;
#pragma unroll
    for (int j = 0; j < BP; ++j) rb[j] = ldg(wt + (size_t)(j * 256 + tid) * VEC);
  };

  const int wave = tid >> 6, lane = tid & 63;
  const int wm = wave / WAVES_N, wn = wave % WAVES_N;
  const int l31 = lane & 31, hi = lane >> 5;
  const int ku_sw = ku ^ ((lrow >> 2) & 3);
  const int sw_r = (l31 >> 2) & 3;
  static_assert(RPP % 16 == 0 && WM % 16 == 0, "swizzle key must not depend on the pass / wave tile");

  f32x16 acc[TM][2];
#pragma unroll
  for (int i = 0; i < TM; ++i)
#pragma unroll
    for (int j = 0; j < 2; ++j)
#pragma unroll
      for (int e = 0; e < 16; ++e) acc[i][j][e] = 0.0f;

  Wide<T, TM> wacc;
  int tap = 0, kc = 0, nxt = 0;
  auto advance = [&]() {
    const bool more = nxt + 1 < niter;
    nxt += more ? 1 : 0;
    const int k2 = kc + 1, wrap = k2 == d.kchunks;
    kc = more ? (wrap ? 0 : k2) : kc;
    tap = more ? tap + wrap : tap;
  };
  gload(ra0, rb0, ok0, tap, kc);
  advance();
  gload(ra1, rb1, ok1, tap, kc);
  advance();
  auto step = [&](stg_t(&ra)[AP], stg_t(&rb)[BP], unsigned& okm, int it) {
    uint4* Ab = As + (it & 1) * BM * PITCH;
    uint4* Bb = Bs + (it & 1) * BN * PITCH;
#pragma unroll
    for (int i = 0; i < AP; ++i) {
      const unsigned m = 0u - ((okm >> i) & 1u);
      *reinterpret_cast<stg_t*>(Ab + (lrow + i * RPP) * PITCH + ku_sw) = ra[i] & m;
    }
#pragma unroll
    for (int j = 0; j < BP; ++j) *reinterpret_cast<stg_t*>(Bb + (lrow + j * RPP) * PITCH + ku_sw) = rb[j];
    __syncthreads();
    gload(ra, rb, okm, tap, kc);
    advance();
    if constexpr (Wide<T>::on) clear_acc<TM>(acc);
#pragma unroll
    for (int call = 0; call < CALLS; ++call) {
      const int unit = Mma<T>::unit_of(call, hi) ^ sw_r;
      typename Mma<T>::Frag fa[TM], fb[2];
#pragma unroll
      for (int i = 0; i < TM; ++i) fa[i] = Mma<T>::load(Ab + (wm * WM + i * 32 + l31) * PITCH + unit);
#pragma unroll
      for (int j = 0; j < 2; ++j) fb[j] = Mma<T>::load(Bb + (wn * 64 + j * 32 + l31) * PITCH + unit);
#pragma unroll
      for (int i = 0; i < TM; ++i)
#pragma unroll
        for (int j = 0; j < 2; ++j) Mma<T>::mma(fa[i], fb[j], acc[i][j], hi);
    }
    wacc.add(acc);
  };
  for (int it = 0; it + 1 < niter; it += 2) {
    step(ra0, rb0, ok0, it);
    step(ra1, rb1, ok1, it + 1);
  }
  if (niter & 1) step(ra0, rb0, ok0, niter - 1);
  wacc.finish(acc);

  if (wide) {
    StatAcc<T> gs, gq;
    auto row_to_m = [&](int r) -> int64_t {
      const int m = tm * BM + wm * WM + r;
      return m < M ? (int64_t)m : (int64_t)-1;
    };
    epilogue_store<T, TM>(L, acc, stage + wave * 32 * 68, lane, tn * BN + wn * 64, row_to_m, gs, gq);
    if (fuse_stats) {
      const int nsplit = HWo / BM;
      const int bimg = (tm * BM) / HWo, slab = tm - bimg * nsplit;
      float* dst = L.gn_partials + ((size_t)bimg * nsplit + slab) * L.gn_groups * 2;
      epilogue_stats<WAVES_M, WAVES_N>(reinterpret_cast<StatAcc<T>*>(stage + 4 * 32 * 68), gs, gq, wave, lane, tn * BN, d.Cout,
                                       L.gn_groups, dst);
    }
  } else {
#pragma unroll
    for (int j = 0; j < 2; ++j) {
      const int col = tn * BN + wn * 64 + j * 32 + l31;
      if (col >= d.Cout) continue;
      const float bv = L.bias ? L.bias[col] : 0.0f;
#pragma unroll
      for (int i = 0; i < TM; ++i)
#pragma unroll
        for (int e = 0; e < 16; ++e) {
          const int row = tm * BM + wm * WM + i * 32 + (e & 3) + 8 * (e >> 2) + 4 * hi;
          if (row < M) {
            float v = acc[i][j][e] + bv;
            const size_t o = (size_t)row * d.Cout + col;
            if (L.residual) v += Elem<T>::load(L.residual[o]);
            L.out[o] = Elem<T>::store(v);
          }
        }
    }
  }
}


template <typename T>
struct HaloPick {
  int TH, TW, BN;
};
template <typename T>
static bool pick_halo(const ConvDesc& d, HaloPick<T>* p) {
  constexpr int CH = 8 * Elem<T>::kVec;
  if (!(d.KH == 3 && d.KW == 3 && d.stride == 1 && d.pad == 1)) return false;
  if (d.C0 % CH || d.C1 % CH || d.Cout % 64) return false;
  const int H = d.Hout, W = d.Wout;
  if (d.Cout % 128 == 0) {
    if (W % 32 == 0 && H % 4 == 0) { *p = {4, 32, 128}; return true; }
    if (W % 16 == 0 && H % 8 == 0) { *p = {8, 16, 128}; return true; }
    return false;
  }
  if (W % 32 == 0 && H % 8 == 0) { *p = {8, 32, 64}; return true; }
  if (W % 16 == 0 && H % 8 == 0) { *p = {8, 16, 64}; return true; }
  return false;
}

template <typename T>
bool conv_supports_prologue(const ConvDesc& d) {
  HaloPick<T> p;
  return d.C1 == 0 && pick_halo<T>(d, &p);
}
template bool conv_supports_prologue<float>(const ConvDesc&);
template bool conv_supports_prologue<bf16_t>(const ConvDesc&);

template <typename T, int TH, int TW, int BN>
static int launch_halo(const ConvLaunch<T>& L, hipStream_t s, int fuse_stats, int* nsplit) {
  const ConvDesc& d = L.d;
  const int tiles_x = d.Wout / TW, tiles_y = d.Hout / TH, tiles_n = d.Cout / BN;
  constexpr int HALO = (TH + 2) * (TW + 2);
  size_t lds = (size_t)(HALO * 8 + 2 * BN * 8) * 16;
  if (lds < kEpilogueLds) lds = kEpilogueLds;
  if (nsplit) *nsplit = fuse_stats ? tiles_x * tiles_y : 0;
  conv3x3_halo_kernel<T, TH, TW, BN><<<dim3(tiles_x * tiles_y * tiles_n * d.B), 256, lds, s>>>(L, tiles_x, tiles_y,
                                                                                            tiles_n, fuse_stats);
  PRG_LAUNCH_CHECK();
  return PRG_OK;
}

template <typename T, int BM, int BN>
static int launch_igemm(const ConvLaunch<T>& L, int M, hipStream_t s, int want_stats, int* nsplit) {
  constexpr int UPR = ConvTile<T>::BK / Elem<T>::kVec;
  const ConvDesc& d = L.d;
  const int tiles_m = ceil_div(M, BM), tiles_n = d.CoutPad / BN;
  const int HWo = d.Hout * d.Wout;
  const int wide = d.Cout % 8 == 0;
  const int cpg = L.gn_groups > 0 ? d.Cout / L.gn_groups : 0;
  const int fuse = want_stats && wide && cpg % 8 == 0 && cpg <= BN && HWo % BM == 0 && HWo / BM <= kGnMaxSplit;
  if (nsplit) *nsplit = fuse ? HWo / BM : 0;
  size_t lds = (size_t)2 * (BM + BN) * UPR * 16;
  if (lds < kEpilogueLds) lds = kEpilogueLds;
  const bool one = d.KH == 1 && d.KW == 1 && d.stride == 1 && d.pad == 0 && !d.ups;
  if (one) conv_igemm_kernel<T, BM, BN, true><<<dim3(tiles_m * tiles_n), 256, lds, s>>>(L, M, tiles_m, tiles_n, fuse, wide);
  else conv_igemm_kernel<T, BM, BN, false><<<dim3(tiles_m * tiles_n), 256, lds, s>>>(L, M, tiles_m, tiles_n, fuse, wide);
  PRG_LAUNCH_CHECK();
  return PRG_OK;
}

template <int TH, int TW, int BN>
static int launch_mx(const ConvLaunch<bf16_t>& L, hipStream_t s, int fuse_stats, int* nsplit) {
  const ConvDesc& d = L.d;
  const int tiles_x = d.Wout / TW, tiles_y = d.Hout / TH, tiles_n = d.Cout / BN;
  constexpr int HALO = (TH + 2) * (TW + 2);
  size_t lds = (size_t)HALO * 80 + (size_t)2 * BN * 80 + ((HALO * 2 + 15) & ~15) + 2 * BN * 2 + 16;
  if (lds < kEpilogueLds) lds = kEpilogueLds;
  if (nsplit) *nsplit = fuse_stats ? tiles_x * tiles_y : 0;
  conv3x3_mx_kernel<TH, TW, BN><<<dim3(tiles_x * tiles_y * tiles_n * d.B), 256, lds, s>>>(L, tiles_x, tiles_y, tiles_n, fuse_stats);
  PRG_LAUNCH_CHECK();
  return PRG_OK;
}
int try_launch_conv3x3_w256mx(const ConvLaunch<bf16_t>& L, hipStream_t s, int* gn_nsplit_out, int* acc_done);
static thread_local double g_last_exec_scale = 1.0;
double conv_last_exec_scale() { return g_last_exec_scale; }
static thread_local int g_last_mx = 0;
int conv_last_was_mx() { return g_last_mx; }

int materialize_prologue(ConvLaunch<bf16_t>& L, hipStream_t s) {
  if (!L.pro_fold.acc) return PRG_OK;
  PRG_CHECK(L.pro_a && L.pro_b, "conv: pro_fold needs scratch coefficient tables in pro_a / pro_b");
  const int rc = launch_gn_coeff_acc(L.pro_fold, const_cast<float*>(L.pro_a), const_cast<float*>(L.pro_b), L.d.B, L.d.C0, s);
  L.pro_fold.acc = nullptr;
  return rc;
}
static int materialize_prologue(ConvLaunch<float>&, hipStream_t) { return PRG_OK; }

static int mx_pure_env() {
  static const int pure = env_int("PRG_MX_PURE", 0);
  return pure;
}
int try_launch_conv3x3_up_w256(const ConvLaunch<bf16_t>& L, hipStream_t s);
static int try_mx(ConvLaunch<bf16_t>& L, hipStream_t s, int* gn_nsplit_out, int* acc_done) {
  if (!L.w_mx || !L.w_mx_scale) return 0;
  if (L.d.ups && !L.gn_partials && !L.mx_pure && !mx_pure_env()) {
    const int r = try_launch_conv3x3_up_w256(L, s);
    if (r == 1) g_last_exec_scale = 4.0 / 9.0;
    if (r != 0) return r;
  }
  {
    const int r = try_launch_conv3x3_w256mx(L, s, gn_nsplit_out, acc_done);
    if (r == 1) g_last_mx = 1;
    if (r != 0) return r;
  }
  if (!mx_pure_env() && !L.mx_pure) return 0;
  const ConvDesc& d = L.d;
  HaloPick<bf16_t> hp;
  if (!pick_halo<bf16_t>(d, &hp) || L.residual) return 0;
  const int cpg = L.gn_groups > 0 ? d.Cout / L.gn_groups : 0;
  const int tiles = (d.Wout / hp.TW) * (d.Hout / hp.TH);
  const int fuse = L.gn_partials != nullptr && cpg % 8 == 0 && cpg <= hp.BN && tiles <= kGnMaxSplit;
  int rc;
  if ((rc = materialize_prologue(L, s))) return rc;
  if (hp.TH == 8 && hp.TW == 32 && hp.BN == 64) rc = launch_mx<8, 32, 64>(L, s, fuse, gn_nsplit_out);
  else if (hp.TH == 4 && hp.TW == 32 && hp.BN == 128) rc = launch_mx<4, 32, 128>(L, s, fuse, gn_nsplit_out);
  else if (hp.TH == 8 && hp.TW == 16 && hp.BN == 128) rc = launch_mx<8, 16, 128>(L, s, fuse, gn_nsplit_out);
  else if (hp.TH == 8 && hp.TW == 16 && hp.BN == 64) rc = launch_mx<8, 16, 64>(L, s, fuse, gn_nsplit_out);
  else return 0;
  if (rc == PRG_OK) g_last_mx = 1;
  return rc == PRG_OK ? 1 : rc;
}
static int try_mx(ConvLaunch<float>&, hipStream_t, int*, int*) { return 0; }

int try_launch_conv3x3_ws(const ConvLaunch<bf16_t>& L, hipStream_t s, int* gn_nsplit_out, int* acc_done);
int try_launch_conv3x3_c64(const ConvLaunch<bf16_t>& L, hipStream_t s, int* gn_nsplit_out, int* acc_done);
int try_launch_conv3x3_w256(const ConvLaunch<bf16_t>& L, hipStream_t s, int* gn_nsplit_out, int* acc_done);
int try_launch_conv4x4s2_w256(const ConvLaunch<bf16_t>& L, hipStream_t s);
int try_launch_conv3x3_up_w256(const ConvLaunch<bf16_t>& L, hipStream_t s);
static inline int try_down(const ConvLaunch<bf16_t>& L, hipStream_t s) { return try_launch_conv4x4s2_w256(L, s); }
static inline int try_down(const ConvLaunch<float>&, hipStream_t) { return 0; }
static inline int try_ws(ConvLaunch<bf16_t>& L, hipStream_t s, int* n, int* acc_done) {
  int r = try_launch_conv3x3_c64(L, s, n, acc_done);
  if (r == 0 && L.d.ups && !L.gn_partials) {
    r = try_launch_conv3x3_up_w256(L, s);
    if (r == 1) g_last_exec_scale = 4.0 / 9.0;
  }
  if (r == 0) r = try_launch_conv3x3_w256(L, s, n, acc_done);
  if (r != 0) return r;
  const ConvDesc& d = L.d;
  if (L.pro_fold.acc && d.KH == 3 && d.KW == 3 && d.stride == 1 && d.pad == 1 && d.C0 % 64 == 0 && d.C1 % 64 == 0 && d.Cout % 64 == 0)
    if (int rc = materialize_prologue(L, s)) return rc;
  return try_launch_conv3x3_ws(L, s, n, acc_done);
}
static inline int try_ws(ConvLaunch<float>&, hipStream_t, int*, int*) { return 0; }
static inline int try_split(const ConvLaunch<float>& L, hipStream_t s, int* n) { return try_launch_conv_split(L, s, n); }
static inline int try_split(const ConvLaunch<bf16_t>&, hipStream_t, int*) { return 0; }

bool conv_h16_pair_ok(const ConvLaunch<bf16_t>& L1in, const ConvLaunch<bf16_t>& L2in) {
  static const int on = env_int("PRG_H16", 1);
  if (!on) return false;
  ConvLaunch<bf16_t> L1 = L1in, L2 = L2in;
  auto mx_takes = [](const ConvLaunch<bf16_t>& L) { return L.w_mx && (L.d.Cout % 128 == 0 || mx_pure_env() || L.mx_pure); };
  if (mx_takes(L1) || mx_takes(L2) || !L2.w_f16 || !L1.gn_acc || !L2.pro_fold.acc) return false;
  L1.probe = L2.probe = 1;
  L1.out_f16 = 1;
  L2.in_f16 = 1;
  int ns = 0, ad = 0;
  int r1 = try_launch_conv3x3_c64(L1, nullptr, &ns, &ad);
  if (r1 == 0) r1 = try_launch_conv3x3_w256(L1, nullptr, &ns, &ad);
  if (r1 == 0) r1 = try_launch_conv3x3_ws(L1, nullptr, &ns, &ad);
  if (r1 != 1 || !ad) return false;
  int r2 = try_launch_conv3x3_c64(L2, nullptr, &ns, &ad);
  if (r2 == 0) r2 = try_launch_conv3x3_w256(L2, nullptr, &ns, &ad);
  return r2 == 1;
}

template <typename T>
int launch_conv(const ConvLaunch<T>& Lin, hipStream_t s, int* gn_nsplit_out, int* acc_done) {
  g_last_exec_scale = 1.0;
  g_last_mx = 0;
  if (acc_done) *acc_done = 0;
  ConvLaunch<T> L = Lin;
  const ConvDesc& d = L.d;
  constexpr int VEC = Elem<T>::kVec;
  PRG_CHECK(L.src0 && L.w && L.out, "conv: null pointer");
  PRG_CHECK(d.C0 % VEC == 0 && d.C1 % VEC == 0, "conv: channel counts must be multiples of the 16-byte vector");
  PRG_CHECK(d.C1 == 0 || L.src1, "conv: second source missing");
  PRG_CHECK(!L.res_a || (L.residual && L.res_b && d.KH == 1 && d.KW == 1 && d.Cout % 8 == 0),
            "conv: the activated residual is a 1x1 (implicit-GEMM, wide epilogue) feature");
  PRG_CHECK(!L.res_fold.acc || (L.residual && d.KH == 1 && d.KW == 1 && d.Cout % 8 == 0 && L.res_fold.cpg % 8 == 0 &&
                                L.res_fold.G * L.res_fold.cpg == d.Cout && L.res_fold.P && L.res_fold.Q),
            "conv: the folded activated residual needs a 1x1 conv whose 8-channel vectors lie inside one GroupNorm group");
  PRG_CHECK(d.CoutPad % 64 == 0 && d.CoutPad >= d.Cout, "conv: bad CoutPad");
  const int64_t M64 = (int64_t)d.B * d.Hout * d.Wout;
  PRG_CHECK(M64 > 0 && M64 < (int64_t)1 << 31, "conv: M out of range");
  const int M = (int)M64;
  const int want_stats = L.gn_partials != nullptr;
  if (gn_nsplit_out) *gn_nsplit_out = 0;
  {
    const int r = try_mx(L, s, gn_nsplit_out, acc_done);
    if (r < 0) return r;
    if (r == 1) return PRG_OK;
  }
  {
    int r = try_ws(L, s, gn_nsplit_out, acc_done);
    if (r == 0 && !L.gn_partials) r = try_down(L, s);
    if (r < 0) return r;
    if (r == 1) return PRG_OK;
  }
  PRG_CHECK(!L.out_f16 && !L.in_f16, "conv: an h16 launch reached a kernel without the f16 format (conv_h16_pair_ok disagrees with the dispatch)");
  if (int rc = materialize_prologue(L, s)) return rc;
  {
    const int r = try_split(L, s, gn_nsplit_out);
    if (r < 0) return r;
    if (r == 1) return PRG_OK;
  }
  HaloPick<T> hp;
  if (pick_halo<T>(d, &hp)) {
    const int cpg = L.gn_groups > 0 ? d.Cout / L.gn_groups : 0;
    const int tiles = (d.Wout / hp.TW) * (d.Hout / hp.TH);
    const int fuse = want_stats && cpg % 8 == 0 && cpg <= hp.BN && tiles <= kGnMaxSplit;
    if (hp.TH == 8 && hp.TW == 32 && hp.BN == 64) return launch_halo<T, 8, 32, 64>(L, s, fuse, gn_nsplit_out);
    if (hp.TH == 4 && hp.TW == 32 && hp.BN == 128) return launch_halo<T, 4, 32, 128>(L, s, fuse, gn_nsplit_out);
    if (hp.TH == 8 && hp.TW == 16 && hp.BN == 128) return launch_halo<T, 8, 16, 128>(L, s, fuse, gn_nsplit_out);
    if (hp.TH == 8 && hp.TW == 16 && hp.BN == 64) return launch_halo<T, 8, 16, 64>(L, s, fuse, gn_nsplit_out);
  }
  PRG_CHECK(!L.pro_a, "conv: fused prologue requested on a shape the halo kernel does not cover");
  if constexpr (std::is_same<T, bf16_t>::value) {
    if (d.CoutPad % 128 == 0 && M % 256 == 0 && (int64_t)(M / 256) * (d.CoutPad / 128) >= (int64_t)2 * 256)
      return launch_igemm<T, 256, 128>(L, M, s, want_stats, gn_nsplit_out);
  }
  if (d.CoutPad % 128 == 0) return launch_igemm<T, 128, 128>(L, M, s, want_stats, gn_nsplit_out);
  if (M >= 256 * 64) return launch_igemm<T, 256, 64>(L, M, s, want_stats, gn_nsplit_out);
  return launch_igemm<T, 128, 64>(L, M, s, want_stats, gn_nsplit_out);
}

void up_equivalent_weights(const float* w, int Cout, int Cin, std::vector<float>& out) {
  out.assign((size_t)4 * Cout * Cin * 4, 0.0f);
  auto slot = [](int dphase, int k) { const int r = dphase + k - 1; return (r >= 0 ? r / 2 : -1) - (dphase - 1); };
  for (int dy = 0; dy < 2; ++dy)
    for (int dx = 0; dx < 2; ++dx)
      for (int o = 0; o < Cout; ++o)
        for (int c = 0; c < Cin; ++c) {
          double acc[2][2] = {{0, 0}, {0, 0}};
          for (int ky = 0; ky < 3; ++ky)
            for (int kx = 0; kx < 3; ++kx) acc[slot(dy, ky)][slot(dx, kx)] += (double)w[(((size_t)o * Cin + c) * 3 + ky) * 3 + kx];
          float* dst = out.data() + ((((size_t)(2 * dy + dx) * Cout + o) * Cin + c) * 4);
          dst[0] = (float)acc[0][0]; dst[1] = (float)acc[0][1]; dst[2] = (float)acc[1][0]; dst[3] = (float)acc[1][1];
        }
}

void s2d_equivalent_weights(const float* w, int Cout, int Cin, std::vector<float>& out) {
  out.assign((size_t)Cout * 4 * Cin * 9, 0.0f);
  for (int o = 0; o < Cout; ++o)
    for (int c = 0; c < Cin; ++c)
      for (int ky = 0; ky < 4; ++ky)
        for (int kx = 0; kx < 4; ++kx) {
          const int by = ky >> 1, dy = ky & 1, bx = kx >> 1, dx = kx & 1;
          const int cv = (2 * dy + dx) * Cin + c;
          out[(((size_t)o * 4 * Cin + cv) * 3 + 1 + by) * 3 + 1 + bx] = w[(((size_t)o * Cin + c) * 4 + ky) * 4 + kx];
        }
}

template int launch_conv<float>(const ConvLaunch<float>&, hipStream_t, int*, int*);
template int launch_conv<bf16_t>(const ConvLaunch<bf16_t>&, hipStream_t, int*, int*);

template <typename T>
void pack_conv_weight(const float* w, int Cout, int Cin, int KH, int KW, std::vector<T>& out, int* CoutPad,
                      int* kchunks) {
  constexpr int BK = ConvTile<T>::BK;
  const int cp = (Cout + 63) / 64 * 64;
  const int kcn = (Cin + BK - 1) / BK;
  out.assign((size_t)KH * KW * kcn * cp * BK, Elem<T>::store(0.0f));
  for (int kh = 0; kh < KH; ++kh)
    for (int kw = 0; kw < KW; ++kw)
      for (int kc = 0; kc < kcn; ++kc)
        for (int n = 0; n < Cout; ++n)
          for (int k = 0; k < BK; ++k) {
            int c = kc * BK + k;
            if (c >= Cin) break;
            float v = w[(((size_t)n * Cin + c) * KH + kh) * KW + kw];
            out[((((size_t)(kh * KW + kw)) * kcn + kc) * cp + n) * BK + k] = Elem<T>::store(v);
          }
  *CoutPad = cp;
  *kchunks = kcn;
}
template void pack_conv_weight<float>(const float*, int, int, int, int, std::vector<float>&, int*, int*);
template void pack_conv_weight<bf16_t>(const float*, int, int, int, int, std::vector<bf16_t>&, int*, int*);

void pack_conv_weight_f16(const float* w, int Cout, int Cin, int KH, int KW, std::vector<uint16_t>& out) {
  constexpr int BK = 32;
  const int cp = (Cout + 63) / 64 * 64;
  const int kcn = (Cin + BK - 1) / BK;
  out.assign((size_t)KH * KW * kcn * cp * BK, 0);
  for (int kh = 0; kh < KH; ++kh)
    for (int kw = 0; kw < KW; ++kw)
      for (int kc = 0; kc < kcn; ++kc)
        for (int n = 0; n < Cout; ++n)
          for (int k = 0; k < BK; ++k) {
            const int c = kc * BK + k;
            if (c >= Cin) break;
            const _Float16 h = (_Float16)w[(((size_t)n * Cin + c) * KH + kh) * KW + kw];
            uint16_t bits;
            std::memcpy(&bits, &h, 2);
            out[((((size_t)(kh * KW + kw)) * kcn + kc) * cp + n) * BK + k] = bits;
          }
}

uint8_t f32_to_e4m3(float v) {
  const uint8_t sign = std::signbit(v) ? 0x80 : 0;
  float a = std::fabs(v);
  if (!(a == a)) return sign | 0x7f;
  if (a >= 448.0f) return sign | 0x7e;
  if (a < 0.0009765625f) return sign;
  int e;
  std::frexp(a, &e);
  int E = e - 1;
  if (E < -6) E = -6;
  const float step = std::ldexp(1.0f, E - 3);
  float q = std::nearbyint(a / step);
  float r = q * step;
  if (r >= 448.0f) return sign | 0x7e;
  if (r < 0.015625f) return sign | (uint8_t)q;
  int e2;
  const float m2 = std::frexp(r, &e2);
  const int Eb = e2 - 1 + 7;
  const int man = (int)std::nearbyint((m2 * 2.0f - 1.0f) * 8.0f);
  return sign | (uint8_t)((Eb << 3) | man);
}
float e4m3_to_f32(uint8_t b) {
  const int s = b >> 7, e = (b >> 3) & 15, m = b & 7;
  const float x = e == 0 ? std::ldexp((float)m, -9) : std::ldexp(1.0f + m / 8.0f, e - 7);
  return s ? -x : x;
}

void pack_conv_weight_mxfp8(const float* w, int Cout, int Cin, int KH, int KW, std::vector<uint8_t>& data,
                            std::vector<uint8_t>& scales, int* CoutPad, int* chunks64) {
  const int cp = (Cout + 63) / 64 * 64, kc = (Cin + 63) / 64;
  data.assign((size_t)KH * KW * kc * cp * 64, 0);
  scales.assign((size_t)KH * KW * kc * cp * 2, 0);
  for (int tap = 0; tap < KH * KW; ++tap)
    for (int c64 = 0; c64 < kc; ++c64)
      for (int n = 0; n < Cout; ++n)
        for (int blk = 0; blk < 2; ++blk) {
          float v[32], am = 0.0f;
          for (int k = 0; k < 32; ++k) {
            const int c = c64 * 64 + blk * 32 + k;
            v[k] = c < Cin ? w[((size_t)n * Cin + c) * KH * KW + tap] : 0.0f;
            am = std::fmax(am, std::fabs(v[k]));
          }
          uint32_t bits;
          std::memcpy(&bits, &am, 4);
          const int E = (int)((bits >> 23) & 0xff);
          const int S = E > 8 ? E - 8 : 0;
          const float mult = std::ldexp(1.0f, 127 - S);
          const size_t row = ((size_t)(tap * kc + c64) * cp + n);
          scales[row * 2 + blk] = (uint8_t)S;
          for (int k = 0; k < 32; ++k) {
            float g = v[k] * mult;
            g = g > 448.0f ? 448.0f : (g < -448.0f ? -448.0f : g);
            data[row * 64 + blk * 32 + k] = f32_to_e4m3(g);
          }
        }
  *CoutPad = cp;
  *chunks64 = kc;
}

template <typename T, int CIN>
__global__ __launch_bounds__(256) void stem_conv_kernel(const float* __restrict__ x, const float* __restrict__ wk,
                                                        const float* __restrict__ bias, T* __restrict__ out, int H,
                                                        int W, int Cout) {
  constexpr int TS = 16, HALO = 3, TW = TS + 2 * HALO;
  __shared__ float tile[CIN * TW * TW];
  const int b = blockIdx.z, ty0 = blockIdx.y * TS, tx0 = blockIdx.x * TS;
  const int tid = threadIdx.x;
  for (int i = tid; i < CIN * TW * TW; i += 256) {
    int c = i / (TW * TW), rem = i - c * TW * TW;
    int yy = ty0 + rem / TW - HALO, xx = tx0 + rem % TW - HALO;
    tile[i] = (yy >= 0 && yy < H && xx >= 0 && xx < W) ? x[((size_t)b * CIN + c) * H * W + (size_t)yy * W + xx] : 0.0f;
  }
  __syncthreads();
  const int ly = tid / TS, lx = tid % TS;
  const int oy = ty0 + ly, ox = tx0 + lx;
  const bool ok = oy < H && ox < W;
  T* o = out + (((size_t)b * H + (ok ? oy : 0)) * W + (ok ? ox : 0)) * Cout;
#pragma unroll 1
  for (int co = 0; co < Cout; co += 8) {
    float acc[8];
#pragma unroll
    for (int u = 0; u < 8; ++u) acc[u] = 0.0f;
#pragma unroll 1
    for (int c = 0; c < CIN; ++c)
#pragma unroll
      for (int kh = 0; kh < 7; ++kh)
#pragma unroll
        for (int kw = 0; kw < 7; ++kw) {
          const float v = tile[c * TW * TW + (ly + kh) * TW + lx + kw];
          const float* wp = wk + ((kh * 7 + kw) * CIN + c) * Cout + co;
#pragma unroll
          for (int u = 0; u < 8; ++u) acc[u] = fmaf(v, wp[u], acc[u]);
        }
    if (ok) {
#pragma unroll
      for (int u = 0; u < 8; ++u) o[co + u] = Elem<T>::store(acc[u] + bias[co + u]);
    }
  }
}

template <typename T>
int launch_stem_conv(const float* x, const float* wk, const float* bias, T* out, int B, int Cin, int H, int W,
                     int Cout, hipStream_t s) {
  PRG_CHECK(Cin == 1 || Cin == 3, "stem conv: Cin must be 1 or 3");
  PRG_CHECK(Cout % 8 == 0, "stem conv: Cout must be a multiple of 8");
  dim3 grid(ceil_div(W, 16), ceil_div(H, 16), B);
  if (Cin == 1)
    stem_conv_kernel<T, 1><<<grid, 256, 0, s>>>(x, wk, bias, out, H, W, Cout);
  else
    stem_conv_kernel<T, 3><<<grid, 256, 0, s>>>(x, wk, bias, out, H, W, Cout);
  PRG_LAUNCH_CHECK();
  return PRG_OK;
}
template int launch_stem_conv<float>(const float*, const float*, const float*, float*, int, int, int, int, int,
                                     hipStream_t);
template int launch_stem_conv<bf16_t>(const float*, const float*, const float*, bf16_t*, int, int, int, int, int,
                                      hipStream_t);

typedef __attribute__((ext_vector_type(8))) __bf16 stem_bf16x8;
typedef __attribute__((ext_vector_type(16))) float stem_f32x16;
__device__ inline uint32_t pack_bf16x2(float a, float b) {
  typedef __attribute__((ext_vector_type(2))) __bf16 bf16x2;
  bf16x2 v = {(__bf16)a, (__bf16)b};
  return __builtin_bit_cast(uint32_t, v);
}

typedef __attribute__((ext_vector_type(8))) _Float16 stem_f16x8;
template <int CIN, bool SPLIT>
__global__ __launch_bounds__(256) void stem_mfma_kernel(const float* __restrict__ x, const uint16_t* __restrict__ wf,
                                                        const float* __restrict__ bias, const float* __restrict__ wscale,
                                                        void* __restrict__ outv, int H, int W) {
  using E = typename std::conditional<SPLIT, _Float16, __bf16>::type;
  using EV = typename std::conditional<SPLIT, stem_f16x8, stem_bf16x8>::type;
  using OT = typename std::conditional<SPLIT, float, uint16_t>::type;
  constexpr int ROWS = 8, PR = ROWS + 7, RC = 40, LDS_ST = SPLIT ? 68 : 72;
  __shared__ float raw[(ROWS + 6) * RC];
  __shared__ __attribute__((aligned(16))) E Ph[PR * 32 * 8];
  __shared__ __attribute__((aligned(16))) E Pl[PR * 32 * 8];
  __shared__ __attribute__((aligned(16))) OT stage[64 * LDS_ST];
  OT* const out = reinterpret_cast<OT*>(outv);
  const int b = blockIdx.z, y0 = blockIdx.y * ROWS, x0 = blockIdx.x * 32, tid = threadIdx.x;
  const int wave = tid >> 6, lane = tid & 63, l31 = lane & 31, hi = lane >> 5;
  const int rt = wave & 1, prow = wave >> 1;
  stem_f32x16 acc[ROWS / 2];
#pragma unroll
  for (int ti = 0; ti < ROWS / 2; ++ti)
#pragma unroll
    for (int e = 0; e < 16; ++e) acc[ti][e] = 0.0f;
#pragma unroll 1
  for (int c = 0; c < CIN; ++c) {
    if (c > 0) __syncthreads();
    for (int i = tid; i < (ROWS + 6) * RC; i += 256) {
      const int r = i / RC, cc = i - r * RC;
      const int yy = y0 - 3 + r, xx = x0 - 4 + cc;
      raw[i] = (yy >= 0 && yy < H && xx >= 0 && xx < W) ? x[(((size_t)b * CIN + c) * H + yy) * W + xx] : 0.0f;
    }
    __syncthreads();
    for (int e = tid; e < PR * 32; e += 256) {
      const int r = e >> 5, p = e & 31;
      EV vh, vl;
#pragma unroll
      for (int j = 0; j < 8; ++j) {
        const float v = r < ROWS + 6 ? raw[r * RC + p + 1 + j] : 0.0f;
        const E h16 = (E)v;
        vh[j] = h16;
        vl[j] = (E)(v - (float)h16);
      }
      *reinterpret_cast<EV*>(Ph + e * 8) = vh;
      *reinterpret_cast<EV*>(Pl + e * 8) = vl;
    }
    EV whi[4], wlo[4];
#pragma unroll
    for (int kk = 0; kk < 4; ++kk) {
      whi[kk] = *reinterpret_cast<const EV*>(wf + (((((size_t)c * 2 + rt) * 2 + 0) * 4 + kk) * 64 + lane) * 8);
      wlo[kk] = *reinterpret_cast<const EV*>(wf + (((((size_t)c * 2 + rt) * 2 + 1) * 4 + kk) * 64 + lane) * 8);
    }
    __syncthreads();
#pragma unroll
    for (int ti = 0; ti < ROWS / 2; ++ti) {
      const int row = 2 * ti + prow;
#pragma unroll
      for (int kk = 0; kk < 4; ++kk) {
        const int pr = row + 2 * kk + hi;
        const EV bh = *reinterpret_cast<const EV*>(Ph + (pr * 32 + l31) * 8);
        const EV bl = *reinterpret_cast<const EV*>(Pl + (pr * 32 + l31) * 8);
        if constexpr (SPLIT) {
          acc[ti] = __builtin_amdgcn_mfma_f32_32x32x16_f16(wlo[kk], bh, acc[ti], 0, 0, 0);
          acc[ti] = __builtin_amdgcn_mfma_f32_32x32x16_f16(whi[kk], bl, acc[ti], 0, 0, 0);
          acc[ti] = __builtin_amdgcn_mfma_f32_32x32x16_f16(whi[kk], bh, acc[ti], 0, 0, 0);
        } else {
          acc[ti] = __builtin_amdgcn_mfma_f32_32x32x16_bf16(wlo[kk], bh, acc[ti], 0, 0, 0);
          acc[ti] = __builtin_amdgcn_mfma_f32_32x32x16_bf16(whi[kk], bl, acc[ti], 0, 0, 0);
          acc[ti] = __builtin_amdgcn_mfma_f32_32x32x16_bf16(whi[kk], bh, acc[ti], 0, 0, 0);
        }
      }
    }
  }
  float bv[16], sv[16];
#pragma unroll
  for (int r = 0; r < 16; ++r) {
    bv[r] = bias[rt * 32 + (r & 3) + 8 * (r >> 2) + 4 * hi];
    sv[r] = SPLIT ? wscale[rt * 32 + (r & 3) + 8 * (r >> 2) + 4 * hi] : 1.0f;
  }
#pragma unroll
  for (int ti = 0; ti < ROWS / 2; ++ti) {
#pragma unroll
    for (int g4 = 0; g4 < 4; ++g4) {
      if constexpr (SPLIT) {
        float4 w;
        w.x = acc[ti][4 * g4] * sv[4 * g4] + bv[4 * g4];
        w.y = acc[ti][4 * g4 + 1] * sv[4 * g4 + 1] + bv[4 * g4 + 1];
        w.z = acc[ti][4 * g4 + 2] * sv[4 * g4 + 2] + bv[4 * g4 + 2];
        w.w = acc[ti][4 * g4 + 3] * sv[4 * g4 + 3] + bv[4 * g4 + 3];
        *reinterpret_cast<float4*>(stage + (prow * 32 + l31) * LDS_ST + rt * 32 + 8 * g4 + 4 * hi) = w;
      } else {
        uint2 w;
        w.x = pack_bf16x2(acc[ti][4 * g4] + bv[4 * g4], acc[ti][4 * g4 + 1] + bv[4 * g4 + 1]);
        w.y = pack_bf16x2(acc[ti][4 * g4 + 2] + bv[4 * g4 + 2], acc[ti][4 * g4 + 3] + bv[4 * g4 + 3]);
        *reinterpret_cast<uint2*>(stage + (prow * 32 + l31) * LDS_ST + rt * 32 + 8 * g4 + 4 * hi) = w;
      }
    }
    __syncthreads();
    constexpr int EPV = SPLIT ? 4 : 8, UPP = 64 / EPV;
#pragma unroll
    for (int i = 0; i < 64 * UPP / 256; ++i) {
      const int v = tid + 256 * i;
      const int px = v / UPP, u = v % UPP;
      const int yy = y0 + 2 * ti + (px >> 5), xx = x0 + (px & 31);
      *reinterpret_cast<uint4*>(out + (((size_t)b * H + yy) * W + xx) * 64 + u * EPV) =
          *reinterpret_cast<const uint4*>(stage + px * LDS_ST + u * EPV);
    }
    __syncthreads();
  }
}

bool stem_conv_mfma_supported(int Cin, int Cout, int H, int W) { return (Cin == 1 || Cin == 3) && Cout == 64 && W % 32 == 0 && H % 8 == 0; }

int launch_stem_conv_mfma(const float* x, const bf16_t* wf, const float* bias, bf16_t* out, int B, int Cin, int H, int W,
                          hipStream_t s) {
  PRG_CHECK(stem_conv_mfma_supported(Cin, 64, H, W) && x && wf && bias && out, "stem conv (MFMA): bad arguments");
  const uint16_t* w16 = reinterpret_cast<const uint16_t*>(wf);
  if (Cin == 1) stem_mfma_kernel<1, false><<<dim3(W / 32, H / 8, B), 256, 0, s>>>(x, w16, bias, nullptr, out, H, W);
  else stem_mfma_kernel<3, false><<<dim3(W / 32, H / 8, B), 256, 0, s>>>(x, w16, bias, nullptr, out, H, W);
  PRG_LAUNCH_CHECK();
  return PRG_OK;
}

int launch_stem_conv_mfma_split(const float* x, const uint16_t* wf, const float* bias, const float* wscale, float* out, int B, int Cin,
                                int H, int W, hipStream_t s) {
  PRG_CHECK(stem_conv_mfma_supported(Cin, 64, H, W) && x && wf && bias && wscale && out, "stem conv (split MFMA): bad arguments");
  if (Cin == 1) stem_mfma_kernel<1, true><<<dim3(W / 32, H / 8, B), 256, 0, s>>>(x, wf, bias, wscale, out, H, W);
  else stem_mfma_kernel<3, true><<<dim3(W / 32, H / 8, B), 256, 0, s>>>(x, wf, bias, wscale, out, H, W);
  PRG_LAUNCH_CHECK();
  return PRG_OK;
}

void pack_stem_mfma_weights(const float* w , int Cin, std::vector<bf16_t>& outv) {
  outv.assign((size_t)Cin * 2 * 2 * 4 * 64 * 8, f32_to_bf16(0.0f));
  for (int c = 0; c < Cin; ++c)
    for (int rt = 0; rt < 2; ++rt)
      for (int kk = 0; kk < 4; ++kk)
        for (int lane = 0; lane < 64; ++lane) {
          const int co = rt * 32 + (lane & 31), kh = 2 * kk + (lane >> 5);
          for (int j = 0; j < 7 && kh < 7; ++j) {
            const float v = w[((size_t)co * Cin + c) * 49 + kh * 7 + j];
            const bf16_t h16 = f32_to_bf16(v);
            const bf16_t l16 = f32_to_bf16(v - bf16_to_f32(h16));
            outv[(((((size_t)c * 2 + rt) * 2 + 0) * 4 + kk) * 64 + lane) * 8 + j] = h16;
            outv[(((((size_t)c * 2 + rt) * 2 + 1) * 4 + kk) * 64 + lane) * 8 + j] = l16;
          }
        }
}

void pack_stem_mfma_weights_split(const float* w , int Cin, std::vector<uint16_t>& outv, std::vector<float>& scale) {
  outv.assign((size_t)Cin * 2 * 2 * 4 * 64 * 8, 0);
  scale.assign(64, 1.0f);
  std::vector<float> mul(64, 1.0f);
  for (int co = 0; co < 64; ++co) {
    float m = 0.0f;
    for (int i = 0; i < Cin * 49; ++i) m = std::fmax(m, std::fabs(w[(size_t)co * Cin * 49 + i]));
    if (m >= 0x1p-100f && std::isfinite(m)) {
      int e = 0;
      (void)std::frexp(m, &e);
      mul[co] = std::ldexp(1.0f, 10 - e);
      scale[co] = std::ldexp(1.0f, e - 10);
    }
  }
  auto bits = [](_Float16 h) { uint16_t u; std::memcpy(&u, &h, 2); return u; };
  for (int c = 0; c < Cin; ++c)
    for (int rt = 0; rt < 2; ++rt)
      for (int kk = 0; kk < 4; ++kk)
        for (int lane = 0; lane < 64; ++lane) {
          const int co = rt * 32 + (lane & 31), kh = 2 * kk + (lane >> 5);
          for (int j = 0; j < 7 && kh < 7; ++j) {
            const float v = w[((size_t)co * Cin + c) * 49 + kh * 7 + j] * mul[co];
            const _Float16 h = (_Float16)v;
            const _Float16 l = (_Float16)(v - (float)h);
            outv[(((((size_t)c * 2 + rt) * 2 + 0) * 4 + kk) * 64 + lane) * 8 + j] = bits(h);
            outv[(((((size_t)c * 2 + rt) * 2 + 1) * 4 + kk) * 64 + lane) * 8 + j] = bits(l);
          }
        }
}

template <typename T>
__global__ void head_conv_kernel(const T* __restrict__ x, const float* __restrict__ w, const float* __restrict__ bias,
                                 float* __restrict__ out, int64_t M, int C, int sigmoid) {
  constexpr int VEC = Elem<T>::kVec;
  const int LP = C / VEC >= 64 ? 64 : (C / VEC >= 32 ? 32 : (C / VEC >= 16 ? 16 : (C / VEC >= 8 ? 8 : (C / VEC >= 4 ? 4 : (C / VEC >= 2 ? 2 : 1)))));
  const int per_block = 256 / LP;
  const int sub = threadIdx.x % LP;
  for (int64_t m = (int64_t)blockIdx.x * per_block + threadIdx.x / LP; m < M; m += (int64_t)gridDim.x * per_block) {
    float acc = 0.0f;
    for (int c = sub * VEC; c < C; c += LP * VEC) {
      Vec16<T> v = vec_load(x + m * C + c);
#pragma unroll
      for (int u = 0; u < VEC; ++u) acc = fmaf(Elem<T>::load(v.e[u]), w[c + u], acc);
    }
    for (int o = LP >> 1; o > 0; o >>= 1) acc += __shfl_xor(acc, o, 64);
    if (sub == 0) {
      float v = acc + bias[0];
      out[m] = sigmoid ? sigmoid_f(v) : v;
    }
  }
}

template <typename T>
int launch_head_conv(const T* x, const float* w, const float* bias, float* out, int64_t M, int C, int sigmoid,
                     hipStream_t s) {
  PRG_CHECK(C % Elem<T>::kVec == 0, "head conv: C must be a multiple of the vector width");
  int grid = (int)((M + 31) / 32);
  if (grid > 8192) grid = 8192;
  head_conv_kernel<T><<<grid, 256, 0, s>>>(x, w, bias, out, M, C, sigmoid);
  PRG_LAUNCH_CHECK();
  return PRG_OK;
}
template int launch_head_conv<float>(const float*, const float*, const float*, float*, int64_t, int, int, hipStream_t);
template int launch_head_conv<bf16_t>(const bf16_t*, const float*, const float*, float*, int64_t, int, int,
                                      hipStream_t);

}
```

### pointreggpt_amd/csrc/unet_debug.hip

```cpp
#include <type_traits>

#include "unet_layout.h"

using namespace prg;

namespace {

template <typename T>
struct DebugConv {
  ConvLaunch<T> L{};
  int Ho = 0, Wo = 0;
  DebugConv(DeviceBuffers& own, const PackedConv<T>& pk, int B, int Cin, int Cout, int H, int W, int K, int stride, int pad, int ups,
            int groups, const char* nomem) {
    Ho = ups ? 2 * H : (H + 2 * pad - K) / stride + 1;
    Wo = ups ? 2 * W : (W + 2 * pad - K) / stride + 1;
    L.d.B = B; L.d.Hin = H; L.d.Win = W; L.d.C0 = Cin; L.d.C1 = 0; L.d.ups = ups; L.d.KH = K; L.d.KW = K; L.d.stride = stride; L.d.pad = pad;
    L.d.Hout = Ho; L.d.Wout = Wo; L.d.Cout = Cout; L.d.CoutPad = pk.CoutPad; L.d.kchunks = pk.kchunks;
    L.gn_groups = groups;
    L.w = own.upload(pk.main, nomem);
    L.w_s2d = own.upload(pk.s2d, nomem); L.s2d_kchunks = pk.s2d_kchunks;
    L.w_up = own.upload(pk.up, nomem);
    L.w_mx = own.upload(pk.mx, nomem); L.w_mx_scale = own.upload(pk.mx_scale, nomem);
    L.w_f16 = own.upload(pk.h16, nomem);
    L.w_split = own.upload(pk.split, nomem); L.split_kchunks = pk.split_kchunks;
    L.split_scale = own.upload(pk.split_scale, nomem);
    L.w_up_split = own.upload(pk.up_split, nomem);
    L.split_scale_up = own.upload(pk.up_split_scale, nomem);
  }
};

template <typename T>
int debug_conv_t(const float* x, const float* w, const float* bias, float* out, int B, int Cin, int Cout, int H, int W, int dtype,
                 int K, int stride, hipStream_t s, int ups) {
  constexpr bool f32 = std::is_same<T, float>::value;
  const char* nomem = f32 ? "prg_debug_conv: hipMalloc failed" : "prg_debug_conv3x3: hipMalloc failed";
  if (dtype == PRG_MXFP8) PRG_CHECK(Cin % 64 == 0 && Cout % 64 == 0, "prg_debug_conv3x3: MX-fp8 needs 64-channel multiples");
  ConvRole role;
  role.upsample = ups != 0;
  const PackedConv<T> pk = pack_conv_host<T>(w, Cout, Cin, K, dtype, role);
  DeviceBuffers own;
  DebugConv<T> c(own, pk, B, Cin, Cout, H, W, K, stride, K == 1 ? 0 : 1, ups, 8, nomem);
  const std::vector<float> zb(Cout, 0.0f);
  T* d_in = own.alloc<T>((size_t)B * H * W * Cin, nomem);
  c.L.src0 = d_in;
  c.L.out = own.alloc<T>((size_t)B * c.Ho * c.Wo * Cout, nomem);
  c.L.bias = own.upload(bias ? bias : zb.data(), (size_t)Cout, nomem);
  c.L.mx_pure = f32 ? 0 : 1;
  if (own.rc) return own.rc;
  int rc = launch_nchw_f32_to_nhwc<T>(x, d_in, B, H * W, Cin, s);
  if (rc == PRG_OK) rc = launch_conv<T>(c.L, s, nullptr);
  if (rc == PRG_OK) rc = launch_nhwc_to_nchw_f32<T>(c.L.out, out, B, c.Ho * c.Wo, Cout, s);
  if (hipStreamSynchronize(s) != hipSuccess && rc == PRG_OK)
    rc = fail(PRG_E_HIP, f32 ? "prg_debug_conv: stream synchronise failed" : "prg_debug_conv3x3: stream synchronise failed");
  return rc;
}

int debug_conv(const float* x, const float* w, const float* bias, float* out, int B, int Cin, int Cout, int H, int W, int dtype, int K,
               int stride, void* stream, int ups = 0) {
  PRG_CHECK(x && w && out, "prg_debug_conv3x3: null pointer");
  PRG_CHECK(B > 0 && H > 0 && W > 0 && Cin % 8 == 0 && Cout % 8 == 0, "prg_debug_conv3x3: bad shape");
  PRG_CHECK(dtype == PRG_BF16 || dtype == PRG_MXFP8 || dtype == PRG_F32 || dtype == PRG_F16X3, "prg_debug_conv3x3: bad dtype");
  hipStream_t s = (hipStream_t)stream;
  if (dtype == PRG_F32 || dtype == PRG_F16X3) return debug_conv_t<float>(x, w, bias, out, B, Cin, Cout, H, W, dtype, K, stride, s, ups);
  return debug_conv_t<bf16_t>(x, w, bias, out, B, Cin, Cout, H, W, dtype, K, stride, s, ups);
}

}

extern "C" {

int prg_debug_block_pair(const float* x, const float* w1, const float* b1, const float* gamma, const float* beta, const float* w2,
                         const float* b2, float* out, int B, int Cin, int C, int H, int W, int groups, int h16, void* stream) {
  PRG_CHECK(x && w1 && b1 && gamma && beta && w2 && b2 && out, "prg_debug_block_pair: null pointer");
  PRG_CHECK(B > 0 && H > 0 && W > 0 && Cin % 64 == 0 && C % 64 == 0 && groups > 0 && C % groups == 0 && (C / groups) % 8 == 0,
            "prg_debug_block_pair: bad shape");
  hipStream_t s = (hipStream_t)stream;
  const char* nomem = "prg_debug_block_pair: hipMalloc failed";
  const size_t M = (size_t)B * H * W;
  ConvRole conv2;
  conv2.conv2 = true;
  const PackedConv<bf16_t> p1 = pack_conv_host<bf16_t>(w1, C, Cin, 3, PRG_BF16, ConvRole{});
  const PackedConv<bf16_t> p2 = pack_conv_host<bf16_t>(w2, C, C, 3, PRG_BF16, conv2);
  std::vector<float> pq(2 * (size_t)C);
  for (int c = 0; c < C; ++c) { pq[c] = gamma[c]; pq[C + c] = beta[c]; }
  DeviceBuffers own;
  DebugConv<bf16_t> c1(own, p1, B, Cin, C, H, W, 3, 1, 1, 0, groups, nomem), c2(own, p2, B, C, C, H, W, 3, 1, 1, 0, groups, nomem);
  ConvLaunch<bf16_t>&L1 = c1.L, &L2 = c2.L;
  const size_t acc_count = (size_t)B * groups * 2;
  bf16_t* d_x = own.alloc<bf16_t>(M * Cin, nomem);
  bf16_t* d_h = own.alloc<bf16_t>(M * C, nomem);
  L1.src0 = d_x; L1.out = d_h; L1.bias = own.upload(b1, (size_t)C, nomem);
  L1.gn_partials = own.alloc<float>((size_t)B * kGnMaxSplit * groups * 2, nomem);
  L1.gn_acc = own.alloc<long long>(acc_count, nomem);
  L2.src0 = d_h; L2.out = own.alloc<bf16_t>(M * C, nomem); L2.bias = own.upload(b2, (size_t)C, nomem);
  GnFold f{};
  f.acc = L1.gn_acc; f.P = own.upload(pq, nomem); f.Q = f.P + C; f.pq_stride = 0;
  f.G = groups; f.cpg = C / groups; f.inv_n = 1.0f / ((float)(H * W) * (float)f.cpg);
  L2.pro_fold = f;
  L2.pro_a = own.alloc<float>((size_t)2 * B * C, nomem); L2.pro_b = L2.pro_a + (size_t)B * C;
  if (own.rc) return own.rc;
  if (hipMemsetAsync(L1.gn_acc, 0, acc_count * sizeof(long long), s) != hipSuccess) return fail(PRG_E_HIP, "prg_debug_block_pair: upload failed");
  int rc = launch_nchw_f32_to_nhwc<bf16_t>(x, d_x, B, H * W, Cin, s);
  if (rc == PRG_OK && h16) {
    if (!conv_h16_pair_ok(L1, L2)) rc = fail(PRG_E_INVALID, "prg_debug_block_pair: the kernels this shape dispatches to do not implement the f16 format");
    L1.out_f16 = 1;
    L2.in_f16 = 1;
  }
  int ns = 0, ad = 0;
  if (rc == PRG_OK) rc = launch_conv<bf16_t>(L1, s, &ns, &ad);
  if (rc == PRG_OK && !ad) rc = fail(PRG_E_INVALID, "prg_debug_block_pair: conv1's kernel does not accumulate fixed-point statistics for this shape");
  if (rc == PRG_OK) rc = launch_conv<bf16_t>(L2, s, nullptr);
  if (rc == PRG_OK) rc = launch_nhwc_to_nchw_f32<bf16_t>(L2.out, out, B, H * W, C, s);
  if (hipStreamSynchronize(s) != hipSuccess && rc == PRG_OK) rc = fail(PRG_E_HIP, "prg_debug_block_pair: stream synchronise failed");
  return rc;
}

int prg_debug_conv3x3(const float* x, const float* w, const float* bias, float* out, int B, int Cin, int Cout, int H, int W,
                      int dtype, void* stream) {
  return debug_conv(x, w, bias, out, B, Cin, Cout, H, W, dtype, 3, 1, stream);
}

int prg_debug_conv(const float* x, const float* w, const float* bias, float* out, int B, int Cin, int Cout, int H, int W,
                   int dtype, int K, int stride, void* stream) {
  PRG_CHECK((K == 1 || K == 3 || K == 4) && (stride == 1 || stride == 2), "prg_debug_conv: K must be 1, 3 or 4, stride 1 or 2");
  PRG_CHECK(dtype == PRG_F32 || dtype == PRG_F16X3 || K != 1, "prg_debug_conv: 1x1 convs only in the float32-storage modes");
  PRG_CHECK(stride == 1 || (H % 2 == 0 && W % 2 == 0), "prg_debug_conv: odd image size");
  return debug_conv(x, w, bias, out, B, Cin, Cout, H, W, dtype, K, stride, stream);
}

int prg_debug_upsample_conv3x3(const float* x, const float* w, const float* bias, float* out, int B, int Cin, int Cout, int H, int W,
                               void* stream) {
  return debug_conv(x, w, bias, out, B, Cin, Cout, H, W, PRG_BF16, 3, 1, stream, 1);
}

int prg_debug_upsample_conv(const float* x, const float* w, const float* bias, float* out, int B, int Cin, int Cout, int H, int W,
                            int dtype, void* stream) {
  return debug_conv(x, w, bias, out, B, Cin, Cout, H, W, dtype, 3, 1, stream, 1);
}

int prg_debug_conv4x4s2(const float* x, const float* w, const float* bias, float* out, int B, int Cin, int Cout, int H, int W,
                        void* stream) {
  PRG_CHECK(H % 2 == 0 && W % 2 == 0, "prg_debug_conv4x4s2: odd image size");
  return debug_conv(x, w, bias, out, B, Cin, Cout, H, W, PRG_BF16, 4, 2, stream);
}

}
```

Before: 14.61 pairs/s.

## Add deep-K 1x1 igemm tiles and a streamed-weight fused attention for C=512

```diff
diff --git a/include/prg.h b/include/prg.h
--- a/include/prg.h
+++ b/include/prg.h
@@ -103,6 +103,7 @@
                         void* stream);
 int prg_debug_conv(const float* x, const float* w, const float* bias, float* out, int B, int Cin, int Cout, int H, int W,
                    int dtype, int K, int stride, void* stream);
+int prg_debug_set_igemm_ks(int ks);
 int prg_debug_upsample_conv(const float* x, const float* w, const float* bias, float* out, int B, int Cin, int Cout, int H, int W,
                             int dtype, void* stream);
 
diff --git a/pointreggpt_amd/_lib.py b/pointreggpt_amd/_lib.py
--- a/pointreggpt_amd/_lib.py
+++ b/pointreggpt_amd/_lib.py
@@ -57,6 +57,7 @@
     "prg_debug_conv4x4s2": (C.c_int, [_P, _P, _P, _P, _I, _I, _I, _I, _I, _P]),
     "prg_debug_conv": (C.c_int, [_P, _P, _P, _P, _I, _I, _I, _I, _I, _I, _I, _I, _P]),
     "prg_debug_upsample_conv": (C.c_int, [_P, _P, _P, _P, _I, _I, _I, _I, _I, _I, _P]),
+    "prg_debug_set_igemm_ks": (C.c_int, [_I]),
     "prg_unet_set_taps": (C.c_int, [_P, _I]),
     "prg_unet_get_tap": (C.c_int, [_P, C.c_char_p, _P, _L, C.POINTER(_I), C.POINTER(_I), C.POINTER(_I), _P]),
     "prg_sampler_create": (C.c_int, [_P, C.POINTER(StepC), _I, _I, _I, C.POINTER(_P)]),
@@ -106,6 +107,9 @@
         fn.argtypes = args
     if lib.prg_abi_version() != 1:
         raise PrgError(f"ABI version mismatch: library {lib.prg_abi_version()}, binding 1")
+    ks = os.environ.get("PRG_IGEMM_KS")
+    if ks and hasattr(lib, "prg_debug_set_igemm_ks") and lib.prg_debug_set_igemm_ks(int(ks)) != 0:
+        raise PrgError(f"PRG_IGEMM_KS={ks}: {lib.prg_last_error().decode()}")
     _lib = lib
     return lib
 
diff --git a/pointreggpt_amd/csrc/attn_fused.hip b/pointreggpt_amd/csrc/attn_fused.hip
--- a/pointreggpt_amd/csrc/attn_fused.hip
+++ b/pointreggpt_amd/csrc/attn_fused.hip
@@ -41,6 +41,8 @@
   static constexpr int LDW = C + 8;
   static constexpr int VPT = C / 32;
   static constexpr int KK = C / 16;
+  static constexpr bool STREAM = C > 256;
+  static constexpr int PF = 8;
 };
 
 __device__ inline float quad_sum(float v) {
@@ -114,6 +116,12 @@
 #pragma unroll
   for (int kk = 0; kk < COLS / 16; ++kk)
     w[kk] = *reinterpret_cast<const bf16x8*>(mat + (size_t)(r0 + l31) * COLS + kk * 16 + hi * 8);
+}
+
+__device__ inline bf16x8 wfrag_g(const bf16_t* p, int kk) { return *reinterpret_cast<const bf16x8*>(p + kk * 16); }
+__device__ inline const bf16_t* per_tile(const bf16_t* p) {
+  asm volatile("" : "+v"(p));
+  return p;
 }
 
 __device__ inline f32x16 zero16() {
@@ -174,9 +182,15 @@
   const int wave = threadIdx.x >> 6, lane = threadIdx.x & 63, l31 = lane & 31, hi = lane >> 5;
   const int ntiles = (N + kTP - 1) / kTP;
   const int tpb = la_tpb(ntiles), t0 = slab * tpb, t1 = min(t0 + tpb, ntiles);
-  bf16x8 wk[G::KK], wv[G::KK];
-  load_wfrags<C>(wk, wqkv, kHid + 32 * wave, l31, hi);
-  load_wfrags<C>(wv, wqkv, 2 * kHid + 32 * wave, l31, hi);
+  constexpr bool STREAM = G::STREAM;
+  constexpr int PF = G::PF;
+  bf16x8 wk[STREAM ? 1 : G::KK], wv[STREAM ? 1 : G::KK];
+  if constexpr (!STREAM) {
+    load_wfrags<C>(wk, wqkv, kHid + 32 * wave, l31, hi);
+    load_wfrags<C>(wv, wqkv, 2 * kHid + 32 * wave, l31, hi);
+  }
+  const bf16_t* wkp = wqkv + (size_t)(kHid + 32 * wave + l31) * C + hi * 8;
+  const bf16_t* wvp = wqkv + (size_t)(2 * kHid + 32 * wave + l31) * C + hi * 8;
   f32x16 kinit0 = zero16();
   if constexpr (!KSTAT) {
     float m = -INFINITY;
@@ -193,19 +207,23 @@
   XTile<C> xt;
   if (t0 < t1) xt.load(x, (int64_t)b * N + (int64_t)t0 * kTP, min(kTP, N - t0 * kTP));
   for (int t = t0; t < t1; ++t) {
+    bf16x8 rk[PF], rv[PF];
+    const bf16_t *wkt = wkp, *wvt = wvp;
+    if constexpr (STREAM) {
+      wkt = per_tile(wkp);
+      wvt = per_tile(wvp);
+#pragma unroll
+      for (int p = 0; p < PF; ++p) {
+        rk[p] = wfrag_g(wkt, p);
+        rv[p] = wfrag_g(wvt, p);
+      }
+    }
     xt.normalize_to(xn);
     __syncthreads();
     if (t + 1 < t1) xt.load(x, (int64_t)b * N + (int64_t)(t + 1) * kTP, min(kTP, N - (t + 1) * kTP));
     const int valid = min(kTP, N - t * kTP);
-    auto half = [&](const int pt, auto full_c) {
+    auto contract = [&](const int pt, const f32x16& k1, const f32x16& v1, auto full_c) {
       constexpr bool FULL = decltype(full_c)::value;
-      f32x16 k1, v1;
-#pragma unroll
-      for (int kk = 0; kk < G::KK; ++kk) {
-        const bf16x8 xf = frag(xn + pt * 32 * G::LDW, G::LDW, l31, hi, kk);
-        k1 = __builtin_amdgcn_mfma_f32_32x32x16_bf16(xf, wk[kk], kk == 0 ? (KSTAT ? zero16() : kinit0) : k1, 0, 0, 0);
-        v1 = __builtin_amdgcn_mfma_f32_32x32x16_bf16(xf, wv[kk], kk == 0 ? zero16() : v1, 0, 0, 0);
-      }
 #pragma unroll
       for (int i = 0; i < 2; ++i) {
         bf16x8 pa, vb;
@@ -222,7 +240,41 @@
         if constexpr (PSUM_MFMA) psum = __builtin_amdgcn_mfma_f32_32x32x16_bf16(pa, ones, psum, 0, 0, 0);
       }
     };
-    if (valid == kTP) {
+    auto half = [&](const int pt, auto full_c) {
+      f32x16 k1, v1;
+#pragma unroll
+      for (int kk = 0; kk < G::KK; ++kk) {
+        const bf16x8 xf = frag(xn + pt * 32 * G::LDW, G::LDW, l31, hi, kk);
+        k1 = __builtin_amdgcn_mfma_f32_32x32x16_bf16(xf, wk[kk], kk == 0 ? (KSTAT ? zero16() : kinit0) : k1, 0, 0, 0);
+        v1 = __builtin_amdgcn_mfma_f32_32x32x16_bf16(xf, wv[kk], kk == 0 ? zero16() : v1, 0, 0, 0);
+      }
+      contract(pt, k1, v1, full_c);
+    };
+    if constexpr (STREAM) {
+      f32x16 k2[2], v2[2];
+#pragma unroll
+      for (int kk = 0; kk < G::KK; ++kk) {
+        const bf16x8 ck = rk[kk % PF], cv = rv[kk % PF];
+        if (kk + PF < G::KK) {
+          rk[kk % PF] = wfrag_g(wkt, kk + PF);
+          rv[kk % PF] = wfrag_g(wvt, kk + PF);
+        }
+#pragma unroll
+        for (int pt = 0; pt < 2; ++pt) {
+          const bf16x8 xf = frag(xn + pt * 32 * G::LDW, G::LDW, l31, hi, kk);
+          k2[pt] = __builtin_amdgcn_mfma_f32_32x32x16_bf16(xf, ck, kk == 0 ? (KSTAT ? zero16() : kinit0) : k2[pt], 0, 0, 0);
+          v2[pt] = __builtin_amdgcn_mfma_f32_32x32x16_bf16(xf, cv, kk == 0 ? zero16() : v2[pt], 0, 0, 0);
+        }
+        if (kk % 8 == 7) __builtin_amdgcn_sched_barrier(0);
+      }
+      if (valid == kTP) {
+        contract(0, k2[0], v2[0], std::true_type{});
+        contract(1, k2[1], v2[1], std::true_type{});
+      } else {
+        contract(0, k2[0], v2[0], std::false_type{});
+        contract(1, k2[1], v2[1], std::false_type{});
+      }
+    } else if (valid == kTP) {
       half(0, std::true_type{});
       half(1, std::true_type{});
     } else {
@@ -290,19 +342,22 @@
   __bf16* xn = reinterpret_cast<__bf16*>(smem);
   __bf16* ot = xn + kTP * G::LDW;
   float* lnb = reinterpret_cast<float*>(ot + kTP * kLdO);
-  __bf16* yt = reinterpret_cast<__bf16*>(lnb + kTP * RTL * 2);
-  float* bias_l = reinterpret_cast<float*>(yt + kTP * G::LDW);
+  constexpr bool STREAM = G::STREAM;
+  constexpr int PF = G::PF;
+  __bf16* yt = STREAM ? xn : reinterpret_cast<__bf16*>(lnb + kTP * RTL * 2);
+  float* bias_l = STREAM ? lnb + kTP * RTL * 2 : reinterpret_cast<float*>(yt + kTP * G::LDW);
   float* outg_l = bias_l + C;
-  if (threadIdx.x < C) {
-    bias_l[threadIdx.x] = bias[threadIdx.x];
-    outg_l[threadIdx.x] = out_g[threadIdx.x];
+  for (int c = threadIdx.x; c < C; c += 256) {
+    bias_l[c] = bias[c];
+    outg_l[c] = out_g[c];
   }
   const int b = blockIdx.y, slab = blockIdx.x;
   const int wave = threadIdx.x >> 6, lane = threadIdx.x & 63, l31 = lane & 31, hi = lane >> 5;
   const int ntiles = (N + kTP - 1) / kTP;
   const int tpb = la_out_tpb(ntiles), t0 = slab * tpb, t1 = min(t0 + tpb, ntiles);
-  bf16x8 wq[G::KK];
-  load_wfrags<C>(wq, wqkv, 32 * wave, l31, hi);
+  bf16x8 wq[STREAM ? 1 : G::KK];
+  if constexpr (!STREAM) load_wfrags<C>(wq, wqkv, 32 * wave, l31, hi);
+  const bf16_t* wqp = wqkv + (size_t)(32 * wave + l31) * C + hi * 8;
   bf16x8 ca[2];
 #pragma unroll
   for (int i = 0; i < 2; ++i)
@@ -314,25 +369,46 @@
     else if (RT <= 4) { yrt[a] = wave; ypt[a] = a; }
     else { yrt[a] = wave * NR + (a >> 1); ypt[a] = a & 1; }
   }
-  bf16x8 wo[NR][kHid / 16];
-#pragma unroll
-  for (int r = 0; r < NR; ++r) load_wfrags<kHid>(wo[r], wout, yrt[RT > 4 ? 2 * r : 0] * 32, l31, hi);
+  bf16x8 wo[STREAM ? 1 : NR][kHid / 16];
+  if constexpr (!STREAM) {
+#pragma unroll
+    for (int r = 0; r < NR; ++r) load_wfrags<kHid>(wo[r], wout, yrt[RT > 4 ? 2 * r : 0] * 32, l31, hi);
+  }
+  const bf16_t* wop = wout + (size_t)(wave * NR * 32 + l31) * kHid + hi * 8;
   XTile<C> xt;
-  if (t0 < t1) xt.load(x, (int64_t)b * N + (int64_t)t0 * kTP, min(kTP, N - t0 * kTP));
+  if (!STREAM && t0 < t1) xt.load(x, (int64_t)b * N + (int64_t)t0 * kTP, min(kTP, N - t0 * kTP));
   for (int t = t0; t < t1; ++t) {
     asm volatile("" ::: "memory");
-    const XTile<C> xraw = xt;
     const int valid = min(kTP, N - t * kTP);
+    bf16x8 rq[PF];
+    const bf16_t *wqt = wqp, *wot = wop;
+    if constexpr (STREAM) {
+      xt.load(x, (int64_t)b * N + (int64_t)t * kTP, valid);
+      wqt = per_tile(wqp);
+      wot = per_tile(wop);
+#pragma unroll
+      for (int p = 0; p < PF; ++p) rq[p] = wfrag_g(wqt, p);
+    }
+    XTile<STREAM ? 32 : C> xraw;
+    if constexpr (!STREAM) xraw = xt;
     xt.normalize_to(xn);
     __syncthreads();
-    if (t + 1 < t1) xt.load(x, (int64_t)b * N + (int64_t)(t + 1) * kTP, min(kTP, N - (t + 1) * kTP));
+    if (!STREAM && t + 1 < t1) xt.load(x, (int64_t)b * N + (int64_t)(t + 1) * kTP, min(kTP, N - (t + 1) * kTP));
     constexpr bool qstat = QSTAT;
     f32x16 qa[2];
 #pragma unroll
     for (int kk = 0; kk < G::KK; ++kk) {
+      bf16x8 cq;
+      if constexpr (STREAM) {
+        cq = rq[kk % PF];
+        if (kk + PF < G::KK) rq[kk % PF] = wfrag_g(wqt, kk + PF);
+        if (kk % 8 == 7) __builtin_amdgcn_sched_barrier(0);
+      } else {
+        cq = wq[kk];
+      }
 #pragma unroll
       for (int pt = 0; pt < 2; ++pt)
-        qa[pt] = __builtin_amdgcn_mfma_f32_32x32x16_bf16(wq[kk], frag(xn + pt * 32 * G::LDW, G::LDW, l31, hi, kk),
+        qa[pt] = __builtin_amdgcn_mfma_f32_32x32x16_bf16(cq, frag(xn + pt * 32 * G::LDW, G::LDW, l31, hi, kk),
                                                          kk == 0 ? zero16() : qa[pt], 0, 0, 0);
     }
 #pragma unroll
@@ -393,12 +469,29 @@
     f32x16 ya[NA];
 #pragma unroll
     for (int a = 0; a < NA; ++a) ya[a] = zero16();
-#pragma unroll
-    for (int kk = 0; kk < kHid / 16; ++kk) {
-#pragma unroll
-      for (int a = 0; a < NA; ++a)
-        ya[a] = __builtin_amdgcn_mfma_f32_32x32x16_bf16(wo[RT > 4 ? (a >> 1) : 0][kk],
-                                                        frag(ot + ypt[a] * 32 * kLdO, kLdO, l31, hi, kk), ya[a], 0, 0, 0);
+    if constexpr (STREAM) {
+      constexpr int KO = kHid / 16, NJ = NR * KO;
+      bf16x8 ro[PF];
+#pragma unroll
+      for (int p = 0; p < PF; ++p) ro[p] = wfrag_g(wot + (size_t)(p / KO) * 32 * kHid, p % KO);
+#pragma unroll
+      for (int j = 0; j < NJ; ++j) {
+        const bf16x8 co = ro[j % PF];
+        if (j + PF < NJ) ro[j % PF] = wfrag_g(wot + (size_t)((j + PF) / KO) * 32 * kHid, (j + PF) % KO);
+#pragma unroll
+        for (int h2 = 0; h2 < 2; ++h2) {
+          const int a = 2 * (j / KO) + h2;
+          ya[a] = __builtin_amdgcn_mfma_f32_32x32x16_bf16(co, frag(ot + ypt[a] * 32 * kLdO, kLdO, l31, hi, j % KO), ya[a], 0, 0, 0);
+        }
+      }
+    } else {
+#pragma unroll
+      for (int kk = 0; kk < kHid / 16; ++kk) {
+#pragma unroll
+        for (int a = 0; a < NA; ++a)
+          ya[a] = __builtin_amdgcn_mfma_f32_32x32x16_bf16(wo[RT > 4 ? (a >> 1) : 0][kk],
+                                                          frag(ot + ypt[a] * 32 * kLdO, kLdO, l31, hi, kk), ya[a], 0, 0, 0);
+      }
     }
 #pragma unroll
     for (int a = 0; a < NA; ++a) {
@@ -443,7 +536,9 @@
 #pragma unroll
         for (int i = 0; i < G::VPT; ++i) {
           const uint4 yv = *reinterpret_cast<const uint4*>(yt + row * G::LDW + (part + 4 * i) * 8);
-          const uint4 xv = xraw.v[i];
+          uint4 xv;
+          if constexpr (STREAM) xv = *reinterpret_cast<const uint4*>(x + ((int64_t)b * N + (int64_t)t * kTP + row) * C + (part + 4 * i) * 8);
+          else xv = xraw.v[i];
           uint4 o;
           o.x = pack2(bf_lo(yv.x) + bf_lo(xv.x), bf_hi(yv.x) + bf_hi(xv.x));
           o.y = pack2(bf_lo(yv.y) + bf_lo(xv.y), bf_hi(yv.y) + bf_hi(xv.y));
@@ -453,6 +548,7 @@
         }
       }
     }
+    if constexpr (STREAM) __syncthreads();
   }
 }
 
@@ -600,7 +696,7 @@
 template <int C>
 size_t lds_kmax() { return (size_t)kTP * Geo<C>::LDW * 2; }
 template <int C>
-size_t lds_out() { return (size_t)2 * kTP * Geo<C>::LDW * 2 + (size_t)kTP * kLdO * 2 + (size_t)kTP * (C / 32 > 4 ? C / 32 : 4) * 2 * 4 + (size_t)2 * C * 4; }
+size_t lds_out() { return (size_t)(Geo<C>::STREAM ? 1 : 2) * kTP * Geo<C>::LDW * 2 + (size_t)kTP * kLdO * 2 + (size_t)kTP * (C / 32 > 4 ? C / 32 : 4) * 2 * 4 + (size_t)2 * C * 4; }
 
 template <typename K>
 int set_lds(K kernel, size_t bytes) {
@@ -854,7 +950,7 @@
   return launch_tail<256, 128>(h, A, Bc, s0, C0, s1, C1, wres, bres, out, B, N, s, f);
 }
 
-bool linattn_fused_supported(int C) { return C == 64 || C == 128 || C == 256; }
+bool linattn_fused_supported(int C) { return C == 64 || C == 128 || C == 256 || C == 512; }
 
 size_t linattn_fused_ws_floats(int B, int N) {
   const size_t ns = la_slabs(N);
@@ -868,6 +964,7 @@
   PRG_CHECK(la_slabs(N) <= 4096, "fused linear attention: too many slabs");
   if (C == 64) return launch_c<64>(x, wqkv, wout, bias, out_g, out, ws, B, N, kshift, s);
   if (C == 256) return launch_c<256>(x, wqkv, wout, bias, out_g, out, ws, B, N, kshift, s);
+  if (C == 512) return launch_c<512>(x, wqkv, wout, bias, out_g, out, ws, B, N, kshift, s);
   return launch_c<128>(x, wqkv, wout, bias, out_g, out, ws, B, N, kshift, s);
 }
 
diff --git a/pointreggpt_amd/csrc/conv.h b/pointreggpt_amd/csrc/conv.h
--- a/pointreggpt_amd/csrc/conv.h
+++ b/pointreggpt_amd/csrc/conv.h
@@ -125,6 +125,7 @@
 
 double conv_last_exec_scale();
 int conv_last_was_mx();
+void conv_set_igemm_ks(int ks);
 
 inline double conv_flops(const ConvDesc& d) {
   return 2.0 * (double)d.B * d.Hout * d.Wout * d.Cout * (double)(d.C0 + d.C1) * d.KH * d.KW;
diff --git a/pointreggpt_amd/csrc/conv.hip b/pointreggpt_amd/csrc/conv.hip
--- a/pointreggpt_amd/csrc/conv.hip
+++ b/pointreggpt_amd/csrc/conv.hip
@@ -1,3 +1,4 @@
+#include <atomic>
 #include <cmath>
 #include <cstdio>
 #include <cstring>
@@ -450,7 +451,7 @@
   }
 }
 
-template <typename T, int BM, int BN, bool ONE>
+template <typename T, int BM, int BN, bool ONE, int KS = 1>
 __global__ __launch_bounds__(256, sizeof(T) == 4 ? 1 : 2) void conv_igemm_kernel(const ConvLaunch<T> L, const int M, const int tiles_m,
                                                          const int tiles_n, const int fuse_stats, const int wide) {
   constexpr int BK = ConvTile<T>::BK;
@@ -462,10 +463,11 @@
   constexpr int WM = BM / WAVES_M, TM = WM / 32;
   constexpr int CALLS = UPR / Mma<T>::UNITS_PER_CALL;
   static_assert(TM >= 1, "wave tile");
+  static_assert(KS == 1 || ONE, "deep K steps are a feature of the 1x1 form");
 
   extern __shared__ __attribute__((aligned(16))) char smem[];
   uint4* As = reinterpret_cast<uint4*>(smem);
-  uint4* Bs = As + 2 * BM * UPR;
+  uint4* Bs = As + 2 * KS * BM * UPR;
   float* stage = reinterpret_cast<float*>(smem);
   constexpr int PITCH = UPR;
   static_assert(UPR == 4, "swizzle assumes 64-byte tile rows");
@@ -504,21 +506,24 @@
 
   typedef __attribute__((ext_vector_type(4))) unsigned int stg_t;
   auto ldg = [](const T* p) { return *reinterpret_cast<const stg_t*>(p); };
-  stg_t ra0[AP], rb0[BP], ra1[AP], rb1[BP];
+  stg_t ra0[KS * AP], rb0[KS * BP], ra1[KS * AP], rb1[KS * BP];
   unsigned ok0 = 0, ok1 = 0;
-  const int niter = d.KH * d.KW * d.kchunks;
-  auto gload = [&](stg_t(&ra)[AP], stg_t(&rb)[BP], unsigned& okm, int tap, int kc) {
+  const int niter = d.KH * d.KW * d.kchunks / KS;
+  auto gload = [&](stg_t(&ra)[KS * AP], stg_t(&rb)[KS * BP], unsigned& okm, int tap, int kc) {
     okm = 0;
     const int kh = tap / d.KW, kw = tap - kh * d.KW;
     const int c = kc * BK + ku * VEC;
     if constexpr (ONE) {
 #pragma unroll
-      for (int i = 0; i < AP; ++i) {
-        const bool ok = a_ok[i] && c < Cin;
-        const T* p = (c < d.C0 ? a_p0[i] : a_p1[i]) + kc * BK;
-        ra[i] = ldg(ok ? p : L.src0);
-        okm |= (ok ? 1u : 0u) << i;
-      }
+      for (int ks = 0; ks < KS; ++ks)
+#pragma unroll
+        for (int i = 0; i < AP; ++i) {
+          const int cs = c + ks * BK;
+          const bool ok = a_ok[i] && cs < Cin;
+          const T* p = (cs < d.C0 ? a_p0[i] : a_p1[i]) + (kc + ks) * BK;
+          ra[ks * AP + i] = ldg(ok ? p : L.src0);
+          okm |= (ok ? 1u : 0u) << (ks * AP + i);
+        }
     } else
 #pragma unroll
     for (int i = 0; i < AP; ++i) {
@@ -532,7 +537,9 @@
     }
     const T* wt = L.w + ((size_t)(tap * d.kchunks + kc) * d.CoutPad + (size_t)tn * BN) * BK;
 #pragma unroll
-    for (int j = 0; j < BP; ++j) rb[j] = ldg(wt + (size_t)(j * 256 + tid) * VEC);
+    for (int ks = 0; ks < KS; ++ks)
+#pragma unroll
+      for (int j = 0; j < BP; ++j) rb[ks * BP + j] = ldg(wt + (size_t)ks * d.CoutPad * BK + (size_t)(j * 256 + tid) * VEC);
   };
 
   const int wave = tid >> 6, lane = tid & 63;
@@ -555,7 +562,7 @@
   auto advance = [&]() {
     const bool more = nxt + 1 < niter;
     nxt += more ? 1 : 0;
-    const int k2 = kc + 1, wrap = k2 == d.kchunks;
+    const int k2 = kc + KS, wrap = k2 == d.kchunks;
     kc = more ? (wrap ? 0 : k2) : kc;
     tap = more ? tap + wrap : tap;
   };
@@ -563,28 +570,33 @@
   advance();
   gload(ra1, rb1, ok1, tap, kc);
   advance();
-  auto step = [&](stg_t(&ra)[AP], stg_t(&rb)[BP], unsigned& okm, int it) {
-    uint4* Ab = As + (it & 1) * BM * PITCH;
-    uint4* Bb = Bs + (it & 1) * BN * PITCH;
-#pragma unroll
-    for (int i = 0; i < AP; ++i) {
-      const unsigned m = 0u - ((okm >> i) & 1u);
-      *reinterpret_cast<stg_t*>(Ab + (lrow + i * RPP) * PITCH + ku_sw) = ra[i] & m;
-    }
-#pragma unroll
-    for (int j = 0; j < BP; ++j) *reinterpret_cast<stg_t*>(Bb + (lrow + j * RPP) * PITCH + ku_sw) = rb[j];
+  auto step = [&](stg_t(&ra)[KS * AP], stg_t(&rb)[KS * BP], unsigned& okm, int it) {
+    uint4* Ab = As + (it & 1) * KS * BM * PITCH;
+    uint4* Bb = Bs + (it & 1) * KS * BN * PITCH;
+#pragma unroll
+    for (int ks = 0; ks < KS; ++ks) {
+#pragma unroll
+      for (int i = 0; i < AP; ++i) {
+        const unsigned m = 0u - ((okm >> (ks * AP + i)) & 1u);
+        *reinterpret_cast<stg_t*>(Ab + (ks * BM + lrow + i * RPP) * PITCH + ku_sw) = ra[ks * AP + i] & m;
+      }
+#pragma unroll
+      for (int j = 0; j < BP; ++j) *reinterpret_cast<stg_t*>(Bb + (ks * BN + lrow + j * RPP) * PITCH + ku_sw) = rb[ks * BP + j];
+    }
     __syncthreads();
     gload(ra, rb, okm, tap, kc);
     advance();
     if constexpr (Wide<T>::on) clear_acc<TM>(acc);
 #pragma unroll
+    for (int ks = 0; ks < KS; ++ks)
+#pragma unroll
     for (int call = 0; call < CALLS; ++call) {
       const int unit = Mma<T>::unit_of(call, hi) ^ sw_r;
       typename Mma<T>::Frag fa[TM], fb[2];
 #pragma unroll
-      for (int i = 0; i < TM; ++i) fa[i] = Mma<T>::load(Ab + (wm * WM + i * 32 + l31) * PITCH + unit);
-#pragma unroll
-      for (int j = 0; j < 2; ++j) fb[j] = Mma<T>::load(Bb + (wn * 64 + j * 32 + l31) * PITCH + unit);
+      for (int i = 0; i < TM; ++i) fa[i] = Mma<T>::load(Ab + (ks * BM + wm * WM + i * 32 + l31) * PITCH + unit);
+#pragma unroll
+      for (int j = 0; j < 2; ++j) fb[j] = Mma<T>::load(Bb + (ks * BN + wn * 64 + j * 32 + l31) * PITCH + unit);
 #pragma unroll
       for (int i = 0; i < TM; ++i)
 #pragma unroll
@@ -678,6 +690,9 @@
   return PRG_OK;
 }
 
+static std::atomic<int> g_igemm_ks_max{2};
+void conv_set_igemm_ks(int ks) { g_igemm_ks_max.store(ks < 1 ? 1 : ks, std::memory_order_relaxed); }
+
 template <typename T, int BM, int BN>
 static int launch_igemm(const ConvLaunch<T>& L, int M, hipStream_t s, int want_stats, int* nsplit) {
   constexpr int UPR = ConvTile<T>::BK / Elem<T>::kVec;
@@ -691,6 +706,21 @@
   size_t lds = (size_t)2 * (BM + BN) * UPR * 16;
   if (lds < kEpilogueLds) lds = kEpilogueLds;
   const bool one = d.KH == 1 && d.KW == 1 && d.stride == 1 && d.pad == 0 && !d.ups;
+  if constexpr (std::is_same<T, bf16_t>::value && BM == 128) {
+    if (one && g_igemm_ks_max.load(std::memory_order_relaxed) >= 2 && d.kchunks % 2 == 0) {
+      constexpr size_t lds2 = (size_t)2 * 2 * (BM + BN) * UPR * 16;
+      static_assert(lds2 >= kEpilogueLds && lds2 <= 64 * 1024, "KS = 2 tile buffers");
+      static DeviceOnce attr_done;
+      if (!attr_done.done()) {
+        PRG_HIP(hipFuncSetAttribute(reinterpret_cast<const void*>(&conv_igemm_kernel<T, BM, BN, true, 2>),
+                                    hipFuncAttributeMaxDynamicSharedMemorySize, (int)lds2));
+        attr_done.mark();
+      }
+      conv_igemm_kernel<T, BM, BN, true, 2><<<dim3(tiles_m * tiles_n), 256, lds2, s>>>(L, M, tiles_m, tiles_n, fuse, wide);
+      PRG_LAUNCH_CHECK();
+      return PRG_OK;
+    }
+  }
   if (one) conv_igemm_kernel<T, BM, BN, true><<<dim3(tiles_m * tiles_n), 256, lds, s>>>(L, M, tiles_m, tiles_n, fuse, wide);
   else conv_igemm_kernel<T, BM, BN, false><<<dim3(tiles_m * tiles_n), 256, lds, s>>>(L, M, tiles_m, tiles_n, fuse, wide);
   PRG_LAUNCH_CHECK();
diff --git a/pointreggpt_amd/csrc/unet_debug.hip b/pointreggpt_amd/csrc/unet_debug.hip
--- a/pointreggpt_amd/csrc/unet_debug.hip
+++ b/pointreggpt_amd/csrc/unet_debug.hip
@@ -123,9 +123,15 @@
 int prg_debug_conv(const float* x, const float* w, const float* bias, float* out, int B, int Cin, int Cout, int H, int W,
                    int dtype, int K, int stride, void* stream) {
   PRG_CHECK((K == 1 || K == 3 || K == 4) && (stride == 1 || stride == 2), "prg_debug_conv: K must be 1, 3 or 4, stride 1 or 2");
-  PRG_CHECK(dtype == PRG_F32 || dtype == PRG_F16X3 || K != 1, "prg_debug_conv: 1x1 convs only in the float32-storage modes");
+  PRG_CHECK(dtype != PRG_MXFP8 || K != 1, "prg_debug_conv: no MX-fp8 1x1 convs");
   PRG_CHECK(stride == 1 || (H % 2 == 0 && W % 2 == 0), "prg_debug_conv: odd image size");
   return debug_conv(x, w, bias, out, B, Cin, Cout, H, W, dtype, K, stride, stream);
+}
+
+int prg_debug_set_igemm_ks(int ks) {
+  PRG_CHECK(ks == 1 || ks == 2, "prg_debug_set_igemm_ks: 1 or 2");
+  conv_set_igemm_ks(ks);
+  return PRG_OK;
 }
 
 int prg_debug_upsample_conv3x3(const float* x, const float* w, const float* bias, float* out, int B, int Cin, int Cout, int H, int W,
```

Result: no change. 14.62 pairs/s (median of 2 runs) (+0.1%).
